# TencentARC/HOSNeRF

Measured on AMD Instinct MI355X. Metric: train rays/sec (stage3: forward + losses + backward + gradient all-reduce + Adam; LPIPS term OFF in this line -- stages.stage3_with_lpips carries it), higher is better.
Workload: dtype f32 (fp16/bf16 hi-lo split MFMA x3, fp32 accumulate)

## Files before the change

hosnerf_amd/csrc/hos_gemm_common.h:

```cpp
#pragma once
#include "hos_common.h"

typedef float f32x16 __attribute__((ext_vector_type(16)));

enum Mode { MODE_FWD = 0, MODE_DGRAD = 1, MODE_WGRAD = 2 };

struct GemmArgs {
    const float* A0; int lda0; int kt0;
    const float* A1; int lda1;
    const float* B;  int ldb;
    float* C; int ldc;
    int M, N;
    int Mload, Nload;
    int red_limit;
    int nk;
    int kt_per_split;
    int tiles_m, tiles_n;
    const float* bias;
    const float* mask; int ldmask;
    float* aux; int aux_col; float p0, p1;
    float* db;
    int accumulate;
    int epi;
    const int* m_dev;
    unsigned int* range_flag;
};

#define HOS_RANGE_LIMIT 6.0e4f


__device__ __forceinline__ bool fwd_epilogue_value(const GemmArgs& a, float& v, int row, int col) {
    switch (a.epi) {
        case HOS_EPI_RELU: v = fmaxf(v, 0.f); break;
        case HOS_EPI_DENSITY: a.aux[row] = softplus_f(v + a.p0); return false;
        case HOS_EPI_RGB: v = sigmoid_f(v) * (1.f + 2.f * a.p0) - a.p0; break;
        case HOS_EPI_NERF_HEAD:
            if (col == a.aux_col) { a.aux[row] = softplus_f(v + a.p0); return false; }
            break;
        case HOS_EPI_SIGMOID_RELU4: v = (col < 3) ? sigmoid_f(v) : fmaxf(v, 0.f); break;
        case HOS_EPI_RESIDUAL: v += a.mask[(size_t)row * a.ldmask + col]; break;
        default: break;
    }
    return true;
}

__device__ __forceinline__ float quad_xor1(float x) {
    return __int_as_float(__builtin_amdgcn_mov_dpp(__float_as_int(x), 0xB1, 0xF, 0xF, true));
}
__device__ __forceinline__ float quad_xor2(float x) {
    return __int_as_float(__builtin_amdgcn_mov_dpp(__float_as_int(x), 0x4E, 0xF, 0xF, true));
}

template <int MODE>
__device__ __forceinline__ void gemm_epilogue_tile(const GemmArgs& a, const f32x16& acc, int row0, int col0, int lane,
                                                   const float4* bias_reg = nullptr, uint32_t* relu_bits = nullptr) {
    const int l31 = lane & 31, lhi = lane >> 5;
    if constexpr (MODE == MODE_WGRAD) {
        const int col = col0 + l31;
        if (col >= a.N) return;
#pragma unroll
        for (int r = 0; r < 16; ++r) {
            const int row = row0 + (r & 3) + 8 * (r >> 2) + 4 * lhi;
            if (row < a.M)
                __hip_atomic_fetch_add(a.C + (size_t)row * a.ldc + col, acc[r], __ATOMIC_RELAXED, __HIP_MEMORY_SCOPE_AGENT);
        }
        return;
    } else {
        const int q = l31 & 3;
        const int colb = col0 + (l31 & ~3);
        const bool c_vec = ((reinterpret_cast<uintptr_t>(a.C) & 15u) == 0) && ((a.ldc & 3) == 0);
        const bool m_vec = a.mask != nullptr && ((reinterpret_cast<uintptr_t>(a.mask) & 15u) == 0) && ((a.ldmask & 3) == 0);
        float4 bias4 = make_float4(0.f, 0.f, 0.f, 0.f);
        bool big = false;
        if (MODE == MODE_FWD && bias_reg != nullptr) bias4 = *bias_reg;
        else if (MODE == MODE_FWD && a.bias != nullptr) {
            if (colb + 0 < a.N) bias4.x = a.bias[colb + 0];
            if (colb + 1 < a.N) bias4.y = a.bias[colb + 1];
            if (colb + 2 < a.N) bias4.z = a.bias[colb + 2];
            if (colb + 3 < a.N) bias4.w = a.bias[colb + 3];
        }
#pragma unroll
        for (int g = 0; g < 4; ++g) {
            float v0 = acc[4 * g + 0], v1 = acc[4 * g + 1], v2 = acc[4 * g + 2], v3 = acc[4 * g + 3];
            {
                const float s0 = (q & 1) ? v0 : v1, s1 = (q & 1) ? v2 : v3;
                const float r0 = quad_xor1(s0), r1 = quad_xor1(s1);
                if (q & 1) { v0 = r0; v2 = r1; } else { v1 = r0; v3 = r1; }
                const float t0 = (q & 2) ? v0 : v2, t1 = (q & 2) ? v1 : v3;
                const float u0 = quad_xor2(t0), u1 = quad_xor2(t1);
                if (q & 2) { v0 = u0; v1 = u1; } else { v2 = u0; v3 = u1; }
            }
            const int row = row0 + q + 8 * g + 4 * lhi;
            if (row >= a.M || colb >= a.N) {
                if (MODE == MODE_FWD && relu_bits != nullptr) *relu_bits <<= 4;
                continue;
            }
            float v[4] = {v0, v1, v2, v3};
            const bool full = colb + 3 < a.N;
            if constexpr (MODE == MODE_FWD) {
                v[0] += bias4.x; v[1] += bias4.y; v[2] += bias4.z; v[3] += bias4.w;
                const bool simple = (a.epi == HOS_EPI_NONE || a.epi == HOS_EPI_RELU);
                if (relu_bits != nullptr) {
                    uint32_t rb = *relu_bits;
#pragma unroll
                    for (int k = 0; k < 4; ++k) rb = __builtin_amdgcn_alignbit(rb, __float_as_uint(0.f - v[k]), 31);
                    *relu_bits = rb;
                }
                if (simple && full && c_vec) {
                    const float pre = (v[0] + v[1]) + (v[2] + v[3]);
                    if (a.epi == HOS_EPI_RELU) { v[0] = fmaxf(v[0], 0.f); v[1] = fmaxf(v[1], 0.f); v[2] = fmaxf(v[2], 0.f); v[3] = fmaxf(v[3], 0.f); }
                    big |= (fmaxf(fmaxf(fabsf(v[0]), fabsf(v[1])), fmaxf(fabsf(v[2]), fabsf(v[3]))) > HOS_RANGE_LIMIT) | (pre != pre);
                    *reinterpret_cast<float4*>(a.C + (size_t)row * a.ldc + colb) = make_float4(v[0], v[1], v[2], v[3]);
                } else {
#pragma unroll
                    for (int k = 0; k < 4; ++k) {
                        const int col = colb + k;
                        if (col >= a.N) break;
                        float x = v[k];
                        if (fwd_epilogue_value(a, x, row, col)) a.C[(size_t)row * a.ldc + col] = x;
                        if (simple) big |= !(fabsf(x) <= HOS_RANGE_LIMIT);
                    }
                }
            } else {
                if (a.mask != nullptr) {
                    if (full && m_vec) {
                        const float4 mk = *reinterpret_cast<const float4*>(a.mask + (size_t)row * a.ldmask + colb);
                        if (!(mk.x > 0.f)) v[0] = 0.f;
                        if (!(mk.y > 0.f)) v[1] = 0.f;
                        if (!(mk.z > 0.f)) v[2] = 0.f;
                        if (!(mk.w > 0.f)) v[3] = 0.f;
                    } else {
#pragma unroll
                        for (int k = 0; k < 4; ++k)
                            if (colb + k < a.N && !(a.mask[(size_t)row * a.ldmask + colb + k] > 0.f)) v[k] = 0.f;
                    }
                }
                float* dst = a.C + (size_t)row * a.ldc + colb;
                if (full && c_vec) {
                    float4 o = make_float4(v[0], v[1], v[2], v[3]);
                    if (a.accumulate) { const float4 p = *reinterpret_cast<const float4*>(dst); o.x += p.x; o.y += p.y; o.z += p.z; o.w += p.w; }
                    *reinterpret_cast<float4*>(dst) = o;
                } else {
#pragma unroll
                    for (int k = 0; k < 4; ++k)
                        if (colb + k < a.N) dst[k] = a.accumulate ? (dst[k] + v[k]) : v[k];
                }
            }
        }
        if (MODE == MODE_FWD && a.range_flag != nullptr && __builtin_amdgcn_ballot_w64(big) != 0 && lane == 0) atomicOr(a.range_flag, 1u);
    }
}

#define HOS_GEMM_FP32 0
#define HOS_GEMM_BF16X3 1
int hos_gemm3_launch(GemmArgs a, int mode, int splits, hipStream_t stream);
```

hosnerf_amd/csrc/hos_mlpbwd.hip:

```cpp
#include "hos_gemm_common.h"
#include <type_traits>
#include <utility>

namespace {

typedef __bf16 bf16x8 __attribute__((ext_vector_type(8)));
typedef __bf16 bf16x4 __attribute__((ext_vector_type(4)));
typedef short s16x4 __attribute__((ext_vector_type(4)));
typedef short s16x8 __attribute__((ext_vector_type(8)));

struct MlpBwdArgs {
    const float* dZ; int lddz;
    const float* X; int ldx;
    const float* W; int ldw;
    float* dX; int lddx;
    float* dW; int lddw;
    float* db;
    int M, N, K;
    int relu_mask;
    float* ws;
    int ws_dw;
    const int* m_dev;
};

constexpr int mb_rows(bool dg) { return dg ? 64 : 32; }
constexpr int MB_NT = 512;

__device__ __forceinline__ float4 ldg4(const float* p) { return *reinterpret_cast<const float4*>(p); }

__device__ __forceinline__ void split4(const float4& v, bf16x4& hi, bf16x4& lo) {
    hi[0] = (__bf16)v.x; hi[1] = (__bf16)v.y; hi[2] = (__bf16)v.z; hi[3] = (__bf16)v.w;
    lo[0] = (__bf16)(v.x - (float)hi[0]); lo[1] = (__bf16)(v.y - (float)hi[1]);
    lo[2] = (__bf16)(v.z - (float)hi[2]); lo[3] = (__bf16)(v.w - (float)hi[3]);
}

__device__ __forceinline__ bf16x8 tr_frag2(const char* p0, int pitch) {
    const s16x4 a = __builtin_amdgcn_ds_read_tr16_b64_v4i16((__attribute__((address_space(3))) s16x4*)(p0));
    const s16x4 b = __builtin_amdgcn_ds_read_tr16_b64_v4i16((__attribute__((address_space(3))) s16x4*)(p0 + 4 * pitch));
    const s16x8 j = __builtin_shufflevector(a, b, 0, 1, 2, 3, 4, 5, 6, 7);
    return __builtin_bit_cast(bf16x8, j);
}

__device__ __forceinline__ f32x16 mma3(const bf16x8& ah, const bf16x8& al, const bf16x8& bh, const bf16x8& bl, f32x16 acc) {
    acc = __builtin_amdgcn_mfma_f32_32x32x16_bf16(al, bh, acc, 0, 0, 0);
    acc = __builtin_amdgcn_mfma_f32_32x32x16_bf16(ah, bl, acc, 0, 0, 0);
    acc = __builtin_amdgcn_mfma_f32_32x32x16_bf16(ah, bh, acc, 0, 0, 0);
    return acc;
}

__device__ __forceinline__ void dgrad_store(const MlpBwdArgs& a, const f32x16& acc, const char* xh_rows, int pitch, int grow0,
                                            int col0, int lane) {
    const int l31 = lane & 31, lhi = lane >> 5, q = l31 & 3;
    const int colb = col0 + (l31 & ~3);
#pragma unroll
    for (int g = 0; g < 4; ++g) {
        float v0 = acc[4 * g + 0], v1 = acc[4 * g + 1], v2 = acc[4 * g + 2], v3 = acc[4 * g + 3];
        {
            const float s0 = (q & 1) ? v0 : v1, s1 = (q & 1) ? v2 : v3;
            const float r0 = quad_xor1(s0), r1 = quad_xor1(s1);
            if (q & 1) { v0 = r0; v2 = r1; } else { v1 = r0; v3 = r1; }
            const float t0 = (q & 2) ? v0 : v2, t1 = (q & 2) ? v1 : v3;
            const float u0 = quad_xor2(t0), u1 = quad_xor2(t1);
            if (q & 2) { v0 = u0; v1 = u1; } else { v2 = u0; v3 = u1; }
        }
        const int lrow = q + 8 * g + 4 * lhi;
        const int row = grow0 + lrow;
        if (row >= a.M || colb >= a.K) continue;
        float v[4] = {v0, v1, v2, v3};
        if (a.relu_mask) {
            const uint2 m = *reinterpret_cast<const uint2*>(xh_rows + lrow * pitch + colb * 2);
            const uint32_t h[4] = {m.x & 0xffffu, m.x >> 16, m.y & 0xffffu, m.y >> 16};
#pragma unroll
            for (int k = 0; k < 4; ++k)
                if ((h[k] & 0x8000u) || (h[k] & 0x7fffu) == 0) v[k] = 0.f;
        }
        float* dst = a.dX + (size_t)row * a.lddx + colb;
        if (colb + 3 < a.K) *reinterpret_cast<float4*>(dst) = make_float4(v[0], v[1], v[2], v[3]);
        else {
#pragma unroll
            for (int k = 0; k < 4; ++k) if (colb + k < a.K) dst[k] = v[k];
        }
    }
}

template <int NT, int KT, bool DG>
__global__ __launch_bounds__(MB_NT, 1) void mlp_bwd_kernel(MlpBwdArgs a) {
    constexpr int N_ = NT * 32, K_ = KT * 32, R = mb_rows(DG);
    if (a.m_dev) a.M = min(a.M, *a.m_dev);
    constexpr int PZ = N_ * 2 + 32, PX = K_ * 2 + 32, PW = K_ * 2 + 32;
    constexpr int W_PLANE = DG ? N_ * PW : 0, Z_PLANE = R * PZ, X_PLANE = R * PX;
    constexpr bool PF2 = DG;
    constexpr int ZU = R * (N_ / 4) / MB_NT, XU = R * (K_ / 4) / MB_NT;
    static_assert(ZU >= 1 && XU >= 1, "tile too small for 512 threads");
    constexpr int DT = DG ? 2 * KT : 0;
    constexpr int WT = NT * KT;
    constexpr int WPW = (WT + 7) / 8;
    static_assert(DT <= 8, "one DGRAD tile per wave");
    static_assert(8 % KT == 0, "a wave's WGRAD tiles share kt");

    extern __shared__ __attribute__((aligned(16))) char smem_mb[];
    char* const Wh = smem_mb;
    char* const Wl = Wh + W_PLANE;
    char* const Zh = Wl + W_PLANE;
    char* const Zl = Zh + Z_PLANE;
    char* const Xh = Zl + Z_PLANE;
    char* const Xl = Xh + X_PLANE;

    const int t = threadIdx.x, lane = t & 63, wave = t >> 6;
    const int l31 = lane & 31, lhi = lane >> 5;
    const int tr_g = lane >> 4, tr_p = lane & 15;
    const int tr_row = 8 * (tr_g >> 1) + (tr_p >> 2);
    const int tr_col = 16 * (tr_g & 1) + 4 * (tr_p & 3);

    float4 rzA[ZU], rxA[XU], rzB[PF2 ? ZU : 1], rxB[PF2 ? XU : 1];
    float4 bsum = make_float4(0.f, 0.f, 0.f, 0.f);
    auto gload = [&](float4 (&rz)[ZU], float4 (&rx)[XU], int rb) {
#pragma unroll
        for (int i = 0; i < ZU; ++i) {
            const int u = t + MB_NT * i, row = u / (N_ / 4), c4 = u % (N_ / 4);
            const int gr = rb * R + row;
            rz[i] = (gr < a.M && c4 * 4 < a.lddz) ? ldg4(a.dZ + (size_t)gr * a.lddz + c4 * 4) : make_float4(0.f, 0.f, 0.f, 0.f);
        }
#pragma unroll
        for (int i = 0; i < XU; ++i) {
            const int u = t + MB_NT * i, row = u / (K_ / 4), c4 = u % (K_ / 4);
            const int gr = rb * R + row;
            rx[i] = (gr < a.M && c4 * 4 < a.K) ? ldg4(a.X + (size_t)gr * a.ldx + c4 * 4) : make_float4(0.f, 0.f, 0.f, 0.f);
        }
    };
    auto sstore = [&](const float4 (&rz)[ZU], const float4 (&rx)[XU]) {
#pragma unroll
        for (int i = 0; i < ZU; ++i) {
            const int u = t + MB_NT * i, row = u / (N_ / 4), c4 = u % (N_ / 4);
            bsum.x += rz[i].x; bsum.y += rz[i].y; bsum.z += rz[i].z; bsum.w += rz[i].w;
            bf16x4 h, l;
            split4(rz[i], h, l);
            *reinterpret_cast<bf16x4*>(Zh + row * PZ + c4 * 8) = h;
            *reinterpret_cast<bf16x4*>(Zl + row * PZ + c4 * 8) = l;
        }
#pragma unroll
        for (int i = 0; i < XU; ++i) {
            const int u = t + MB_NT * i, row = u / (K_ / 4), c4 = u % (K_ / 4);
            bf16x4 h, l;
            split4(rx[i], h, l);
            *reinterpret_cast<bf16x4*>(Xh + row * PX + c4 * 8) = h;
            *reinterpret_cast<bf16x4*>(Xl + row * PX + c4 * 8) = l;
        }
    };

    f32x16 accW[WPW];
#pragma unroll
    for (int j = 0; j < WPW; ++j)
#pragma unroll
        for (int r = 0; r < 16; ++r) accW[j][r] = 0.f;

    const int nrb = (a.M + R - 1) / R;
    const int G = gridDim.x;
    auto compute = [&](int rb) {
        f32x16 acc;
        const int rt = wave / KT, kt = wave % KT;
        if constexpr (DG) if (wave < DT) {
#pragma unroll
            for (int r = 0; r < 16; ++r) acc[r] = 0.f;
            const char* zrow = Zh + (rt * 32 + l31) * PZ + lhi * 16;
            const char* wfrag = Wh + tr_row * PW + (kt * 32 + tr_col) * 2;
#pragma unroll
            for (int s = 0; s < N_ / 16; ++s) {
                const bf16x8 ah = *reinterpret_cast<const bf16x8*>(zrow + s * 32);
                const bf16x8 al = *reinterpret_cast<const bf16x8*>(zrow + Z_PLANE + s * 32);
                const bf16x8 bh = tr_frag2(wfrag + s * 16 * PW, PW);
                const bf16x8 bl = tr_frag2(wfrag + W_PLANE + s * 16 * PW, PW);
                acc = mma3(ah, al, bh, bl, acc);
            }
        }
        if (wave < WT) {
            const int kw = wave % KT;
            const char* xfrag = Xh + tr_row * PX + (kw * 32 + tr_col) * 2;
#pragma unroll
            for (int s = 0; s < R / 16; ++s) {
                const bf16x8 bh = tr_frag2(xfrag + s * 16 * PX, PX);
                const bf16x8 bl = tr_frag2(xfrag + X_PLANE + s * 16 * PX, PX);
#pragma unroll
                for (int j = 0; j < WPW; ++j) {
                    const int ti = wave + 8 * j;
                    if (ti < WT) {
                        const char* zfrag = Zh + tr_row * PZ + ((ti / KT) * 32 + tr_col) * 2;
                        const bf16x8 ah = tr_frag2(zfrag + s * 16 * PZ, PZ);
                        const bf16x8 al = tr_frag2(zfrag + Z_PLANE + s * 16 * PZ, PZ);
                        accW[j] = mma3(ah, al, bh, bl, accW[j]);
                    }
                }
            }
        }
        if constexpr (DG) if (wave < DT && a.dX != nullptr) dgrad_store(a, acc, Xh + rt * 32 * PX, PX, rb * R + rt * 32, kt * 32, lane);
    };

    int rb = blockIdx.x;
    if (rb < nrb) gload(rzA, rxA, rb);
    if constexpr (PF2) if (rb + G < nrb) gload(rzB, rxB, rb + G);
    if constexpr (DG) {
        constexpr int WU = N_ * (K_ / 4) / MB_NT;
        float4 rw[WU];
#pragma unroll
        for (int i = 0; i < WU; ++i) {
            const int u = t + MB_NT * i, row = u / (K_ / 4), c4 = u % (K_ / 4);
            rw[i] = (row < a.N && c4 * 4 < a.K) ? ldg4(a.W + (size_t)row * a.ldw + c4 * 4) : make_float4(0.f, 0.f, 0.f, 0.f);
        }
#pragma unroll
        for (int i = 0; i < WU; ++i) {
            const int u = t + MB_NT * i, row = u / (K_ / 4), c4 = u % (K_ / 4);
            bf16x4 h, l;
            split4(rw[i], h, l);
            *reinterpret_cast<bf16x4*>(Wh + row * PW + c4 * 8) = h;
            *reinterpret_cast<bf16x4*>(Wl + row * PW + c4 * 8) = l;
        }
    }
    if constexpr (PF2) {
        while (rb < nrb) {
            sstore(rzA, rxA);
            __syncthreads();
            if (rb + 2 * G < nrb) gload(rzA, rxA, rb + 2 * G);
            compute(rb);
            __syncthreads();
            rb += G;
            if (rb >= nrb) break;
            sstore(rzB, rxB);
            __syncthreads();
            if (rb + 2 * G < nrb) gload(rzB, rxB, rb + 2 * G);
            compute(rb);
            __syncthreads();
            rb += G;
        }
    } else {
        for (; rb < nrb; rb += G) {
            sstore(rzA, rxA);
            __syncthreads();
            if (rb + G < nrb) gload(rzA, rxA, rb + G);
            compute(rb);
            __syncthreads();
        }
    }

    GemmArgs ew{};
    if (a.ws != nullptr && a.ws_dw) {
        ew.C = a.ws + (size_t)blockIdx.x * (N_ * K_ + N_); ew.ldc = K_; ew.M = N_; ew.N = K_; ew.epi = HOS_EPI_NONE;
#pragma unroll
        for (int j = 0; j < WPW; ++j) {
            const int ti = wave + 8 * j;
            if (ti < WT) gemm_epilogue_tile<MODE_FWD>(ew, accW[j], (ti / KT) * 32, (ti % KT) * 32, lane);
        }
    } else {
        ew.C = a.dW; ew.ldc = a.lddw; ew.M = a.N; ew.N = a.K;
#pragma unroll
        for (int j = 0; j < WPW; ++j) {
            const int ti = wave + 8 * j;
            if (ti < WT) gemm_epilogue_tile<MODE_WGRAD>(ew, accW[j], (ti / KT) * 32, (ti % KT) * 32, lane);
        }
    }
    if (a.db != nullptr) {
        float4* red = reinterpret_cast<float4*>(Zh);
        red[t] = bsum;
        __syncthreads();
        constexpr int G = N_ / 4;
        if (t < G) {
            float4 s = make_float4(0.f, 0.f, 0.f, 0.f);
            for (int k = t; k < MB_NT; k += G) { const float4 v = red[k]; s.x += v.x; s.y += v.y; s.z += v.z; s.w += v.w; }
            const float sv[4] = {s.x, s.y, s.z, s.w};
            bool direct = true;
            if (a.ws != nullptr) {
                const int nk = a.ws_dw ? N_ * K_ : 0;
                *reinterpret_cast<float4*>(a.ws + (size_t)blockIdx.x * (nk + N_) + nk + t * 4) = s;
                direct = false;
            }
            if (direct) {
#pragma unroll
                for (int q = 0; q < 4; ++q)
                    if (t * 4 + q < a.N) __hip_atomic_fetch_add(a.db + t * 4 + q, sv[q], __ATOMIC_RELAXED, __HIP_MEMORY_SCOPE_AGENT);
            }
        }
    }
}

template <int KT>
__global__ __launch_bounds__(MB_NT, 1) void wgrad_tr_fast_kernel(MlpBwdArgs a) {
    constexpr int NT = 8, N_ = NT * 32, K_ = KT * 32, R = 32;
    constexpr int PZ = N_ * 2 + 32, PX = K_ * 2 + 32;
    constexpr int Z_PLANE = R * PZ, X_PLANE = R * PX;
    constexpr int ZU = R * (N_ / 4) / MB_NT;
    constexpr int XT = R * (K_ / 4);
    constexpr int XU = (XT + MB_NT - 1) / MB_NT;
    constexpr bool XALL = XT % MB_NT == 0;
    constexpr int WT = NT * KT, WPW = WT / 8;
    static_assert(WT % 8 == 0 && 8 % KT == 0, "a wave's WGRAD tiles share kt");

    extern __shared__ __attribute__((aligned(16))) char smem_mb[];
    char* const Zh = smem_mb;
    char* const Zl = Zh + Z_PLANE;
    char* const Xh = Zl + Z_PLANE;
    char* const Xl = Xh + X_PLANE;
    const int t = threadIdx.x, lane = t & 63, wave = t >> 6;
    const int tr_g = lane >> 4, tr_p = lane & 15;
    const int tr_row = 8 * (tr_g >> 1) + (tr_p >> 2);
    const int tr_col = 16 * (tr_g & 1) + 4 * (tr_p & 3);
    const bool xthread = XALL || t < XT;

    const int nrb = (a.m_dev ? min(a.M, *a.m_dev) : a.M) / R;
    const int G = gridDim.x;
    float4 rzA[ZU], rxA[XU], rzB[ZU], rxB[XU];
    float4 bsum = make_float4(0.f, 0.f, 0.f, 0.f);
    auto gload = [&](float4 (&rz)[ZU], float4 (&rx)[XU], int rb) {
        rb = rb < nrb ? rb : nrb - 1;
        const float* zb = a.dZ + (size_t)rb * R * a.lddz;
        const float* xb = a.X + (size_t)rb * R * a.ldx;
#pragma unroll
        for (int i = 0; i < ZU; ++i) {
            const int u = t + MB_NT * i, row = u / (N_ / 4), c4 = u % (N_ / 4);
            rz[i] = ldg4(zb + (size_t)row * a.lddz + c4 * 4);
        }
#pragma unroll
        for (int i = 0; i < XU; ++i) {
            const int u = XALL ? t + MB_NT * i : (t < XT ? t : 0), row = u / (K_ / 4), c4 = u % (K_ / 4);
            rx[i] = ldg4(xb + (size_t)row * a.ldx + c4 * 4);
        }
    };
    auto sstore = [&](const float4 (&rz)[ZU], const float4 (&rx)[XU]) {
#pragma unroll
        for (int i = 0; i < ZU; ++i) {
            const int u = t + MB_NT * i, row = u / (N_ / 4), c4 = u % (N_ / 4);
            bsum.x += rz[i].x; bsum.y += rz[i].y; bsum.z += rz[i].z; bsum.w += rz[i].w;
            bf16x4 h, l;
            split4(rz[i], h, l);
            *reinterpret_cast<bf16x4*>(Zh + row * PZ + c4 * 8) = h;
            *reinterpret_cast<bf16x4*>(Zl + row * PZ + c4 * 8) = l;
        }
        if (xthread) {
#pragma unroll
            for (int i = 0; i < XU; ++i) {
                const int u = t + MB_NT * i, row = u / (K_ / 4), c4 = u % (K_ / 4);
                bf16x4 h, l;
                split4(rx[i], h, l);
                *reinterpret_cast<bf16x4*>(Xh + row * PX + c4 * 8) = h;
                *reinterpret_cast<bf16x4*>(Xl + row * PX + c4 * 8) = l;
            }
        }
    };
    f32x16 accW[WPW];
#pragma unroll
    for (int j = 0; j < WPW; ++j)
#pragma unroll
        for (int r = 0; r < 16; ++r) accW[j][r] = 0.f;
    auto compute = [&]() {
        const int kw = wave % KT;
        const char* xfrag = Xh + tr_row * PX + (kw * 32 + tr_col) * 2;
#pragma unroll
        for (int s = 0; s < R / 16; ++s) {
            const bf16x8 bh = tr_frag2(xfrag + s * 16 * PX, PX);
            const bf16x8 bl = tr_frag2(xfrag + X_PLANE + s * 16 * PX, PX);
#pragma unroll
            for (int j = 0; j < WPW; ++j) {
                const int ti = wave + 8 * j;
                const char* zfrag = Zh + tr_row * PZ + ((ti / KT) * 32 + tr_col) * 2;
                const bf16x8 ah = tr_frag2(zfrag + s * 16 * PZ, PZ);
                const bf16x8 al = tr_frag2(zfrag + Z_PLANE + s * 16 * PZ, PZ);
                accW[j] = mma3(ah, al, bh, bl, accW[j]);
            }
        }
    };
#define WG_BAR() asm volatile("s_waitcnt lgkmcnt(0)\n\ts_barrier" ::: "memory")
    auto step = [&](float4 (&rz)[ZU], float4 (&rx)[XU], const int rb) {
        sstore(rz, rx);
        WG_BAR();
        gload(rz, rx, rb + 2 * G);
        compute();
        WG_BAR();
    };
    int rb = blockIdx.x;
    if (rb < nrb) {
        gload(rzA, rxA, rb);
        gload(rzB, rxB, rb + G);
        step(rzA, rxA, rb);
        rb += G;
        if (rb < nrb) {
            step(rzB, rxB, rb);
            rb += G;
            while (rb + G < nrb) {
                step(rzA, rxA, rb);
                step(rzB, rxB, rb + G);
                rb += 2 * G;
            }
            if (rb < nrb) step(rzA, rxA, rb);
        }
    }
#undef WG_BAR
    GemmArgs ew{};
    ew.C = a.ws + (size_t)blockIdx.x * (N_ * K_ + N_); ew.ldc = K_; ew.M = N_; ew.N = K_; ew.epi = HOS_EPI_NONE;
#pragma unroll
    for (int j = 0; j < WPW; ++j) {
        const int ti = wave + 8 * j;
        gemm_epilogue_tile<MODE_FWD>(ew, accW[j], (ti / KT) * 32, (ti % KT) * 32, lane);
    }
    if (a.db != nullptr) {
        float4* red = reinterpret_cast<float4*>(Zh);
        red[t] = bsum;
        __syncthreads();
        constexpr int CG = N_ / 4;
        if (t < CG) {
            float4 sacc = make_float4(0.f, 0.f, 0.f, 0.f);
            for (int k = t; k < MB_NT; k += CG) { const float4 v = red[k]; sacc.x += v.x; sacc.y += v.y; sacc.z += v.z; sacc.w += v.w; }
            *reinterpret_cast<float4*>(a.ws + (size_t)blockIdx.x * (N_ * K_ + N_) + N_ * K_ + t * 4) = sacc;
        }
    }
}

constexpr int MB_RSPLIT = 2;
__global__ __launch_bounds__(256) void mlp_bwd_reduce_kernel(const float* __restrict__ ws, int slabs, int n_, int k_, int nk, float* __restrict__ dW,
                                                             int lddw, float* __restrict__ db, int N, int K) {
    const int e = (blockIdx.x * 256 + threadIdx.x) * 4;
    const int slab = nk + n_;
    if (e >= slab || (e >= nk && db == nullptr)) return;
    float4 s = make_float4(0.f, 0.f, 0.f, 0.f);
    const int sy = gridDim.y;
    for (int g0 = blockIdx.y; g0 < slabs; g0 += 8 * sy) {
        float4 v[8];
#pragma unroll
        for (int i = 0; i < 8; ++i) {
            const int g = g0 + i * sy;
            v[i] = g < slabs ? *reinterpret_cast<const float4*>(ws + (size_t)g * slab + e) : make_float4(0.f, 0.f, 0.f, 0.f);
        }
#pragma unroll
        for (int i = 0; i < 8; ++i) { s.x += v[i].x; s.y += v[i].y; s.z += v[i].z; s.w += v[i].w; }
    }
    const float sv[4] = {s.x, s.y, s.z, s.w};
    if (e >= nk) {
#pragma unroll
        for (int q = 0; q < 4; ++q)
            if (e - nk + q < N) __hip_atomic_fetch_add(db + e - nk + q, sv[q], __ATOMIC_RELAXED, __HIP_MEMORY_SCOPE_AGENT);
        return;
    }
    const int n = e / k_, k = e % k_;
    if (n < N) {
#pragma unroll
        for (int q = 0; q < 4; ++q)
            if (k + q < K) __hip_atomic_fetch_add(dW + (size_t)n * lddw + k + q, sv[q], __ATOMIC_RELAXED, __HIP_MEMORY_SCOPE_AGENT);
    }
}

constexpr int MB_BATCH = 16;
struct ReduceJob { const float* ws; float* dW; float* db; int slabs, n_, k_, nk, lddw, N, K, first_block; };
struct ReduceBatch { ReduceJob j[MB_BATCH]; int count; };

__global__ __launch_bounds__(256) void mlp_bwd_reduce_batch_kernel(const ReduceBatch b) {
    int ji = 0;
#pragma unroll 1
    for (int i = 1; i < b.count; ++i) if ((int)blockIdx.x >= b.j[i].first_block) ji = i;
    const ReduceJob& J = b.j[ji];
    const int e = (((int)blockIdx.x - J.first_block) * 256 + threadIdx.x) * 4;
    const int slab = J.nk + J.n_;
    if (e >= slab || (e >= J.nk && J.db == nullptr)) return;
    float4 s = make_float4(0.f, 0.f, 0.f, 0.f);
    const int sy = gridDim.y;
    for (int g0 = blockIdx.y; g0 < J.slabs; g0 += 8 * sy) {
        float4 v[8];
#pragma unroll
        for (int i = 0; i < 8; ++i) {
            const int g = g0 + i * sy;
            v[i] = g < J.slabs ? *reinterpret_cast<const float4*>(J.ws + (size_t)g * slab + e) : make_float4(0.f, 0.f, 0.f, 0.f);
        }
#pragma unroll
        for (int i = 0; i < 8; ++i) { s.x += v[i].x; s.y += v[i].y; s.z += v[i].z; s.w += v[i].w; }
    }
    const float sv[4] = {s.x, s.y, s.z, s.w};
    if (e >= J.nk) {
#pragma unroll
        for (int q = 0; q < 4; ++q)
            if (e - J.nk + q < J.N) __hip_atomic_fetch_add(J.db + e - J.nk + q, sv[q], __ATOMIC_RELAXED, __HIP_MEMORY_SCOPE_AGENT);
        return;
    }
    const int n = e / J.k_, k = e % J.k_;
    if (n < J.N) {
#pragma unroll
        for (int q = 0; q < 4; ++q)
            if (k + q < J.K) __hip_atomic_fetch_add(J.dW + (size_t)n * J.lddw + k + q, sv[q], __ATOMIC_RELAXED, __HIP_MEMORY_SCOPE_AGENT);
    }
}

thread_local bool g_defer = false;
thread_local ReduceBatch g_batch = {};

static int flush_reduce_batch(hipStream_t stream) {
    if (g_batch.count == 0) return 0;
    const ReduceJob& L = g_batch.j[g_batch.count - 1];
    const int blocks = L.first_block + hos_cdiv(L.nk + L.n_, 1024);
    hipLaunchKernelGGL(mlp_bwd_reduce_batch_kernel, dim3(blocks, MB_RSPLIT), dim3(256), 0, stream, g_batch);
    g_batch.count = 0;
    return hos_launch_status();
}

template <int NT, int KT, bool DG>
int launch_mb(MlpBwdArgs a, size_t ws_floats, hipStream_t stream) {
    constexpr int N_ = NT * 32, K_ = KT * 32;
    constexpr int R = mb_rows(DG);
    constexpr size_t smem = (DG ? 2 * (size_t)N_ * (K_ * 2 + 32) : 0) + 2 * (size_t)R * (N_ * 2 + 32) + 2 * (size_t)R * (K_ * 2 + 32);
    static bool attr_set = false;
    if (!attr_set) {
        hipError_t e = hipFuncSetAttribute(reinterpret_cast<const void*>(&mlp_bwd_kernel<NT, KT, DG>),
                                           hipFuncAttributeMaxDynamicSharedMemorySize, (int)smem);
        if (e != hipSuccess) return (int)e;
        attr_set = true;
    }
    const int nrb = hos_cdiv(a.M, R);
    const int grid = nrb < 256 ? nrb : 256;
    a.ws_dw = 1;
    const int nk = a.ws_dw ? N_ * K_ : 0;
    if (a.ws != nullptr && (grid < 32 || ws_floats < (size_t)grid * (nk + N_) || (!a.ws_dw && a.db == nullptr))) a.ws = nullptr;
    hipLaunchKernelGGL((mlp_bwd_kernel<NT, KT, DG>), dim3(grid), dim3(MB_NT), smem, stream, a);
    if (a.ws != nullptr) {
        if (g_defer) {
            if (g_batch.count == MB_BATCH) { const int rc = flush_reduce_batch(stream); if (rc != 0) return rc; }
            ReduceJob& J = g_batch.j[g_batch.count];
            J = ReduceJob{a.ws, a.dW, a.db, grid, N_, K_, nk, a.lddw, a.N, a.K,
                          g_batch.count ? g_batch.j[g_batch.count - 1].first_block + hos_cdiv(g_batch.j[g_batch.count - 1].nk + g_batch.j[g_batch.count - 1].n_, 1024) : 0};
            ++g_batch.count;
        } else {
            hipLaunchKernelGGL(mlp_bwd_reduce_kernel, dim3(hos_cdiv(nk + N_, 1024), MB_RSPLIT), dim3(256), 0, stream,
                               a.ws, grid, N_, K_, nk, a.dW, a.lddw, a.db, a.N, a.K);
        }
    }
    return hos_launch_status();
}

template <int KT>
int launch_wgrad_fast(MlpBwdArgs a, size_t ws_floats, hipStream_t stream) {
    constexpr int N_ = 256, K_ = KT * 32, R = 32, nk = N_ * K_;
    constexpr size_t smem = 2 * (size_t)R * (N_ * 2 + 32) + 2 * (size_t)R * (K_ * 2 + 32);
    const int nrb = a.M / R;
    const int grid = nrb < 256 ? nrb : 256;
    if (a.M % R != 0 || a.N != N_ || a.K != K_ || a.ws == nullptr || grid < 32 ||
        ws_floats < (size_t)grid * (nk + N_) || (((uintptr_t)a.ws) & 15u)) return -1;
    static bool attr_set = false;
    if (!attr_set) {
        hipError_t e = hipFuncSetAttribute(reinterpret_cast<const void*>(&wgrad_tr_fast_kernel<KT>), hipFuncAttributeMaxDynamicSharedMemorySize, (int)smem);
        if (e != hipSuccess) return (int)e;
        attr_set = true;
    }
    hipLaunchKernelGGL((wgrad_tr_fast_kernel<KT>), dim3(grid), dim3(MB_NT), smem, stream, a);
    if (g_defer) {
        if (g_batch.count == MB_BATCH) { const int rc = flush_reduce_batch(stream); if (rc != 0) return rc; }
        ReduceJob& J = g_batch.j[g_batch.count];
        J = ReduceJob{a.ws, a.dW, a.db, grid, N_, K_, nk, a.lddw, a.N, a.K,
                      g_batch.count ? g_batch.j[g_batch.count - 1].first_block + hos_cdiv(g_batch.j[g_batch.count - 1].nk + g_batch.j[g_batch.count - 1].n_, 1024) : 0};
        ++g_batch.count;
    } else {
        hipLaunchKernelGGL(mlp_bwd_reduce_kernel, dim3(hos_cdiv(nk + N_, 1024), MB_RSPLIT), dim3(256), 0, stream,
                           a.ws, grid, N_, K_, nk, a.dW, a.lddw, a.db, a.N, a.K);
    }
    return hos_launch_status();
}

template <int NT, int KT, bool DG>
int64_t ws_floats_mb(int M) {
    const int nrb = hos_cdiv(M, mb_rows(DG));
    const int grid = nrb < 256 ? nrb : 256;
    return grid < 32 ? 0 : (int64_t)grid * (NT * 32 * KT * 32 + NT * 32);
}


typedef unsigned int u32x4 __attribute__((ext_vector_type(4)));
constexpr int CB_MAXS = 4;
constexpr int CB_R = 64;
constexpr int CB_W_BYTES = 2 * 128 * (128 * 2 + 32);
constexpr int CB_T_BYTES = 2 * CB_R * (128 * 2 + 32);
constexpr int CB_SMEM = CB_W_BYTES + 2 * CB_T_BYTES;

constexpr int cb_code(int nt, int kt, int mask, int out) { return nt | (kt << 4) | (mask << 8) | (out << 9); }
constexpr int cb_nt(int c) { return c & 15; }
constexpr int cb_kt(int c) { return (c >> 4) & 15; }
constexpr bool cb_mask(int c) { return (c >> 8) & 1; }
constexpr bool cb_out(int c) { return (c >> 9) & 1; }
constexpr int cb_image_bytes(int nt, int kt) { return ((2 * nt * 32 * (kt * 64 + 32)) + 8191) / 8192 * 8192; }

struct ChainBwdStep {
    const float* X; int ldx;
    const u32x4* Wp;
    float* dXout; int lddx;
    float* ws;
};
struct ChainBwdArgs {
    const float* dZ; int lddz;
    int M; const int* m_dev;
    ChainBwdStep st[CB_MAXS];
};

template <class F, int... I>
__device__ __forceinline__ void cb_static_for(F&& f, std::integer_sequence<int, I...>) { (f(std::integral_constant<int, I>{}), ...); }

template <int... CODE>
__global__ __launch_bounds__(MB_NT, 1) void chain_bwd_kernel(ChainBwdArgs a) {
    constexpr int S = sizeof...(CODE);
    constexpr int codes[S] = {CODE...};
    static_assert(S >= 1 && S <= CB_MAXS && cb_out(codes[S - 1]), "the last step of a group hands its dX over through HBM");
    constexpr int R = CB_R;
    constexpr auto wpw = [](int s) constexpr { return (cb_nt(codes[s]) * cb_kt(codes[s]) + 7) / 8; };
    constexpr auto acc_off = [wpw](int s) constexpr { int o = 0; for (int i = 0; i < s; ++i) o += wpw(i); return o; };
    constexpr int NACC = acc_off(S);
    constexpr auto zsrc = [](int s) constexpr { int v = -1; for (int i = 0; i < s; ++i) if (!cb_out(codes[i])) v = i; return v; };

    if (a.m_dev) a.M = min(a.M, *a.m_dev);
    extern __shared__ __attribute__((aligned(16))) char smem_mb[];
    char* const Wh = smem_mb;
    char* const Zh = smem_mb + CB_W_BYTES;
    char* const Xh = Zh + CB_T_BYTES;
    const int t = threadIdx.x, lane = t & 63, wave = t >> 6;
    const int l31 = lane & 31, lhi = lane >> 5;
    const int tr_g = lane >> 4, tr_p = lane & 15;
    const int tr_row = 8 * (tr_g >> 1) + (tr_p >> 2);
    const int tr_col = 16 * (tr_g & 1) + 4 * (tr_p & 3);

    constexpr int N0 = cb_nt(codes[0]) * 32;
    constexpr int ZU0 = R * (N0 / 4) / MB_NT;
    float4 rz[ZU0];
    float4 rx[4];
    u32x4 rw[9];
    float4 bsum = make_float4(0.f, 0.f, 0.f, 0.f);
    float4 zsum[S];
    f32x16 accW[NACC];
#pragma unroll
    for (int j = 0; j < NACC; ++j)
#pragma unroll
        for (int r = 0; r < 16; ++r) accW[j][r] = 0.f;
#pragma unroll
    for (int s = 0; s < S; ++s) zsum[s] = make_float4(0.f, 0.f, 0.f, 0.f);

    const int nrb = (a.M + R - 1) / R;
    const int G = gridDim.x;
    const int mlast = a.M - 1;

    auto uni = [](const void* p) {
        const uint64_t v = reinterpret_cast<uint64_t>(p);
        const uint32_t lo = __builtin_amdgcn_readfirstlane((uint32_t)v), hi = __builtin_amdgcn_readfirstlane((uint32_t)(v >> 32));
        return reinterpret_cast<const char*>(((uint64_t)hi << 32) | lo);
    };
    auto blk_rlast = [&](int rb) { return min(R - 1, mlast - rb * R); };
    auto gloadZ = [&](int rb) {
        rb = rb < nrb ? rb : nrb - 1;
        const char* base = uni(a.dZ + (size_t)rb * R * a.lddz);
        const int rlast = blk_rlast(rb);
#pragma unroll
        for (int i = 0; i < ZU0; ++i) {
            const int u = t + MB_NT * i, row = min(u / (N0 / 4), rlast), c4 = u % (N0 / 4);
            rz[i] = *reinterpret_cast<const float4*>(base + (unsigned)((row * a.lddz + c4 * 4) * 4));
        }
    };
    auto sstoreZ = [&](int rb) {
        constexpr int PZ = N0 * 2 + 32;
#pragma unroll
        for (int i = 0; i < ZU0; ++i) {
            const int u = t + MB_NT * i, row = u / (N0 / 4), c4 = u % (N0 / 4);
            float4 v = rz[i];
            if (rb * R + row >= a.M) v = make_float4(0.f, 0.f, 0.f, 0.f);
            bsum.x += v.x; bsum.y += v.y; bsum.z += v.z; bsum.w += v.w;
            bf16x4 h, l;
            split4(v, h, l);
            *reinterpret_cast<bf16x4*>(Zh + row * PZ + c4 * 8) = h;
            *reinterpret_cast<bf16x4*>(Zh + R * PZ + row * PZ + c4 * 8) = l;
        }
    };
    auto gloadX_part = [&](auto sc, int rb, int i0, int i1) {
        constexpr int s = decltype(sc)::value;
        constexpr int K_ = cb_kt(codes[s]) * 32, XU = R * (K_ / 4) / MB_NT;
        rb = rb < nrb ? rb : nrb - 1;
        const int ldx = a.st[s].ldx;
        const char* base = uni(a.st[s].X + (size_t)rb * R * ldx);
        const int rlast = blk_rlast(rb);
#pragma unroll
        for (int i = 0; i < XU; ++i) if (i >= i0 && i < i1) {
            const int u = t + MB_NT * i, row = min(u / (K_ / 4), rlast), c4 = u % (K_ / 4);
            rx[i] = *reinterpret_cast<const float4*>(base + (unsigned)((row * ldx + c4 * 4) * 4));
        }
    };
    auto gloadX = [&](auto sc, int rb) { gloadX_part(sc, rb, 0, 4); };
    auto sstoreX = [&](auto sc) {
        constexpr int s = decltype(sc)::value;
        constexpr int K_ = cb_kt(codes[s]) * 32, XU = R * (K_ / 4) / MB_NT, PX = K_ * 2 + 32;
#pragma unroll
        for (int i = 0; i < XU; ++i) {
            const int u = t + MB_NT * i, row = u / (K_ / 4), c4 = u % (K_ / 4);
            bf16x4 h, l;
            split4(rx[i], h, l);
            *reinterpret_cast<bf16x4*>(Xh + row * PX + c4 * 8) = h;
            *reinterpret_cast<bf16x4*>(Xh + R * PX + row * PX + c4 * 8) = l;
        }
    };
    const unsigned toff = (unsigned)t * 16u;
    auto loadW_part = [&](auto sc, int i0, int i1) {
        constexpr int s = decltype(sc)::value;
        constexpr int RW = cb_image_bytes(cb_nt(codes[s]), cb_kt(codes[s])) / 8192;
#pragma unroll
        for (int i = 0; i < RW; ++i) if (i >= i0 && i < i1) rw[i] = *reinterpret_cast<const u32x4*>(uni(reinterpret_cast<const char*>(a.st[s].Wp) + (size_t)i * 8192) + toff);
// ... 120 lines not shown
                    if (wave < DT) {
                        const int q = l31 & 3;
                        const int colb = kt * 32 + (l31 & ~3);
#pragma unroll
                        for (int g = 0; g < 4; ++g) {
                            const int lrow = rt * 32 + q + 8 * g + 4 * lhi;
                            bf16x4 h, l;
                            split4(make_float4(v[g][0], v[g][1], v[g][2], v[g][3]), h, l);
                            *reinterpret_cast<bf16x4*>(Zh + lrow * PZn + colb * 2) = h;
                            *reinterpret_cast<bf16x4*>(Zh + R * PZn + lrow * PZn + colb * 2) = l;
                        }
                    }
                }
                sstoreX(std::integral_constant<int, s + 1 < S ? s + 1 : 0>{});
                storeW(std::integral_constant<int, s + 1 < S ? s + 1 : 0>{});
                __syncthreads();
            }
        }, std::make_integer_sequence<int, S>{});
        __syncthreads();
    }

    cb_static_for([&](auto sc) {
        constexpr int s = decltype(sc)::value;
        constexpr int NT = cb_nt(codes[s]), KT = cb_kt(codes[s]), N_ = NT * 32, K_ = KT * 32;
        constexpr int WT = NT * KT, WPW = (WT + 7) / 8;
        GemmArgs ew{};
        ew.C = a.st[s].ws + (size_t)blockIdx.x * (N_ * K_ + N_); ew.ldc = K_; ew.M = N_; ew.N = K_; ew.epi = HOS_EPI_NONE;
#pragma unroll
        for (int j = 0; j < WPW; ++j) {
            const int ti = wave + 8 * j;
            if (ti < WT) gemm_epilogue_tile<MODE_FWD>(ew, accW[acc_off(s) + j], (ti / KT) * 32, (ti % KT) * 32, lane);
        }
    }, std::make_integer_sequence<int, S>{});
    float4* red = reinterpret_cast<float4*>(Zh);
    {
        red[t] = bsum;
        __syncthreads();
        constexpr int CG = N0 / 4;
        float4 sacc = make_float4(0.f, 0.f, 0.f, 0.f);
        if (t < CG)
            for (int k = t; k < MB_NT; k += CG) { const float4 x = red[k]; sacc.x += x.x; sacc.y += x.y; sacc.z += x.z; sacc.w += x.w; }
        cb_static_for([&](auto sc) {
            constexpr int s = decltype(sc)::value;
            constexpr int N_ = cb_nt(codes[s]) * 32, K_ = cb_kt(codes[s]) * 32;
            if constexpr (zsrc(s) == -1)
                if (t < CG) *reinterpret_cast<float4*>(a.st[s].ws + (size_t)blockIdx.x * (N_ * K_ + N_) + N_ * K_ + t * 4) = sacc;
        }, std::make_integer_sequence<int, S>{});
        __syncthreads();
    }
    cb_static_for([&](auto pc) {
        constexpr int p = decltype(pc)::value;
        if constexpr (!cb_out(codes[p])) {
            constexpr int KTp = cb_kt(codes[p]), CG = KTp * 8;
            red[t] = (wave < 2 * KTp) ? zsum[p] : make_float4(0.f, 0.f, 0.f, 0.f);
            __syncthreads();
            float4 sacc = make_float4(0.f, 0.f, 0.f, 0.f);
            if (t < CG) {
                const int kt = t >> 3, cq = t & 7;
#pragma unroll
                for (int rt = 0; rt < 2; ++rt)
#pragma unroll
                    for (int hh = 0; hh < 2; ++hh)
#pragma unroll
                        for (int q = 0; q < 4; ++q) {
                            const float4 x = red[(rt * KTp + kt) * 64 + hh * 32 + cq * 4 + q];
                            sacc.x += x.x; sacc.y += x.y; sacc.z += x.z; sacc.w += x.w;
                        }
            }
            cb_static_for([&](auto sc) {
                constexpr int s = decltype(sc)::value;
                constexpr int N_ = cb_nt(codes[s]) * 32, K_ = cb_kt(codes[s]) * 32;
                if constexpr (zsrc(s) == p)
                    if (t < CG) *reinterpret_cast<float4*>(a.st[s].ws + (size_t)blockIdx.x * (N_ * K_ + N_) + N_ * K_ + t * 4) = sacc;
            }, std::make_integer_sequence<int, S>{});
            __syncthreads();
        }
    }, std::make_integer_sequence<int, S>{});
}

struct ChainBwdPackJob { const float* W; int ldw, N, K, nt, kt; uint16_t* image; };
struct ChainBwdPackJobs { ChainBwdPackJob j[8]; };
__global__ __launch_bounds__(256) void chain_bwd_pack_kernel(const ChainBwdPackJobs jobs) {
    const ChainBwdPackJob& J = jobs.j[blockIdx.y];
    const int N_ = J.nt * 32, K_ = J.kt * 32, pw = K_ + 16;
    const int total = cb_image_bytes(J.nt, J.kt) / 2;
    for (int e = blockIdx.x * 256 + threadIdx.x; e < total; e += gridDim.x * 256) {
        const int plane = e / (N_ * pw), r = e % (N_ * pw);
        const int n = r / pw, k = r % pw;
        uint16_t out = 0;
        if (plane < 2 && n < J.N && k < J.K) {
            const float w = J.W[(size_t)n * J.ldw + k];
            const __bf16 hi = (__bf16)w;
            out = plane == 0 ? __builtin_bit_cast(uint16_t, hi) : __builtin_bit_cast(uint16_t, (__bf16)(w - (float)hi));
        }
        J.image[e] = out;
    }
}

struct ChainBwdCfg { int S; int code[CB_MAXS]; };
constexpr int CB_NCFG = 4;
constexpr ChainBwdCfg CB_CFG[CB_NCFG] = {
    {2, {cb_code(1, 4, 1, 0), cb_code(4, 4, 1, 1), 0, 0}},
    {3, {cb_code(4, 2, 0, 1), cb_code(4, 4, 1, 0), cb_code(4, 4, 1, 1), 0}},
    {3, {cb_code(4, 4, 1, 0), cb_code(4, 4, 1, 0), cb_code(4, 2, 0, 1), 0}},
    {3, {cb_code(4, 4, 1, 0), cb_code(4, 4, 1, 0), cb_code(4, 4, 0, 1), 0}},
};

template <int... CODE>
int launch_chain_bwd(const ChainBwdArgs& a, int grid, hipStream_t stream) {
    static bool attr_set = false;
    if (!attr_set) {
        hipError_t e = hipFuncSetAttribute(reinterpret_cast<const void*>(&chain_bwd_kernel<CODE...>), hipFuncAttributeMaxDynamicSharedMemorySize, CB_SMEM);
        if (e != hipSuccess) return (int)e;
        attr_set = true;
    }
    hipLaunchKernelGGL((chain_bwd_kernel<CODE...>), dim3(grid), dim3(MB_NT), CB_SMEM, stream, a);
    return hos_launch_status();
}

}

extern "C" int hos_linear_bwd_fused(const float* dZ, int lddz, const float* X, int ldx, const float* W, int ldw,
                                    float* dX, int lddx, float* dW, int lddw, float* db, int M, int N, int K,
                                    int relu_mask, float* ws, int64_t ws_floats, const int32_t* rows_dev, hos_stream_t stream) {
    if (!dZ || !X || !W || !dW || M <= 0 || N <= 0 || K <= 0 || ws_floats < 0) return HOS_E_ARG;
    if (N > 128 || K > 128) return HOS_E_SHAPE;
    if ((lddz & 3) || (ldx & 3) || (ldw & 3) || (K & 3) || (dX && (lddx & 3))) return HOS_E_ALIGN;
    if (((uintptr_t)dZ | (uintptr_t)X | (uintptr_t)W | (uintptr_t)ws) & 15u) return HOS_E_ALIGN;
    MlpBwdArgs a{dZ, lddz, X, ldx, W, ldw, dX, lddx, dW, lddw, db, M, N, K, relu_mask, ws, 1, rows_dev};
    hipStream_t s = static_cast<hipStream_t>(stream);
    const int nt = hos_cdiv(N, 32), kt = hos_cdiv(K, 32);
    if (nt <= 1 && kt <= 4) return launch_mb<1, 4, true>(a, (size_t)ws_floats, s);
    if (kt <= 2) return launch_mb<4, 2, true>(a, (size_t)ws_floats, s);
    return launch_mb<4, 4, true>(a, (size_t)ws_floats, s);
}

extern "C" int hos_linear_wgrad_tr(const float* dZ, int lddz, const float* X, int ldx, float* dW, int lddw, float* db,
                                   int M, int N, int K, float* ws, int64_t ws_floats, const int32_t* rows_dev, hos_stream_t stream) {
    if (!dZ || !X || !dW || M <= 0 || N <= 0 || K <= 0) return HOS_E_ARG;
    if (N > 256 || K > 256) return HOS_E_SHAPE;
    if ((lddz & 3) || (ldx & 3) || (K & 3)) return HOS_E_ALIGN;
    if (((uintptr_t)dZ | (uintptr_t)X) & 15u) return HOS_E_ALIGN;
    MlpBwdArgs a{dZ, lddz, X, ldx, nullptr, 0, nullptr, 0, dW, lddw, db, M, N, K, 0, ws, 0, rows_dev};
    hipStream_t s = static_cast<hipStream_t>(stream);
    const int kt = hos_cdiv(K, 32);
    if (N == 256 && (K == 256 || K == 64)) {
        const int rc = K == 256 ? launch_wgrad_fast<8>(a, (size_t)ws_floats, s) : launch_wgrad_fast<2>(a, (size_t)ws_floats, s);
        if (rc >= 0) return rc;
    }
    if (kt <= 4) return launch_mb<8, 4, false>(a, (size_t)ws_floats, s);
    return launch_mb<8, 8, false>(a, (size_t)ws_floats, s);
}

extern "C" int hos_mlp_bwd_defer(int on) { g_defer = on != 0; return 0; }

extern "C" int hos_mlp_bwd_flush(hos_stream_t stream) { return flush_reduce_batch(static_cast<hipStream_t>(stream)); }

extern "C" long long hos_mlp_bwd_ws_floats(int M, int N, int K, int fused) {
    if (M <= 0 || N <= 0 || K <= 0) return 0;
    const int nt = hos_cdiv(N, 32), kt = hos_cdiv(K, 32);
    if (fused) {
        if (nt <= 1 && kt <= 4) return ws_floats_mb<1, 4, true>(M);
        if (kt <= 2) return ws_floats_mb<4, 2, true>(M);
        return ws_floats_mb<4, 4, true>(M);
    }
    return kt <= 4 ? ws_floats_mb<8, 4, false>(M) : ws_floats_mb<8, 8, false>(M);
}

extern "C" int hos_mlp_chain_bwd_steps(int cfg) { return cfg >= 0 && cfg < CB_NCFG ? CB_CFG[cfg].S : HOS_E_ARG; }

extern "C" long long hos_mlp_chain_bwd_image_bytes(int cfg, int step) {
    if (cfg < 0 || cfg >= CB_NCFG || step < 0 || step >= CB_CFG[cfg].S) return 0;
    return cb_image_bytes(cb_nt(CB_CFG[cfg].code[step]), cb_kt(CB_CFG[cfg].code[step]));
}

extern "C" long long hos_mlp_chain_bwd_ws_floats(int cfg, int M) {
    if (cfg < 0 || cfg >= CB_NCFG || M <= 0) return 0;
    const int nrb = hos_cdiv(M, CB_R), grid = nrb < 256 ? nrb : 256;
    long long f = 0;
    for (int s = 0; s < CB_CFG[cfg].S; ++s) {
        const int n_ = cb_nt(CB_CFG[cfg].code[s]) * 32, k_ = cb_kt(CB_CFG[cfg].code[s]) * 32;
        f += (long long)grid * (n_ * k_ + n_);
    }
    return f;
}

extern "C" int hos_mlp_chain_bwd_pack(int n, const int* cfg, const int* step, const float* const* W, const int* ldw, const int* N,
                                      const int* K, void* const* image, hos_stream_t stream) {
    if (n <= 0 || n > 8 || !cfg || !step || !W || !ldw || !N || !K || !image) return HOS_E_ARG;
    ChainBwdPackJobs jobs{};
    for (int i = 0; i < n; ++i) {
        if (cfg[i] < 0 || cfg[i] >= CB_NCFG || step[i] < 0 || step[i] >= CB_CFG[cfg[i]].S || !W[i] || !image[i] || N[i] <= 0 || K[i] <= 0) return HOS_E_ARG;
        const int nt = cb_nt(CB_CFG[cfg[i]].code[step[i]]), kt = cb_kt(CB_CFG[cfg[i]].code[step[i]]);
        if (N[i] > nt * 32 || K[i] > kt * 32 || ldw[i] < K[i]) return HOS_E_SHAPE;
        if ((uintptr_t)image[i] & 15u) return HOS_E_ALIGN;
        jobs.j[i] = ChainBwdPackJob{W[i], ldw[i], N[i], K[i], nt, kt, static_cast<uint16_t*>(image[i])};
    }
    hipLaunchKernelGGL(chain_bwd_pack_kernel, dim3(36, n), dim3(256), 0, static_cast<hipStream_t>(stream), jobs);
    return hos_launch_status();
}

extern "C" int hos_mlp_chain_bwd(int cfg, const float* dZ, int lddz, int M, const int32_t* rows_dev, const float* const* X, const int* ldx,
                                 const void* const* images, float* const* dXout, const int* lddx, float* const* dW, const int* lddw,
                                 float* const* db, const int* N, const int* K, float* ws, int64_t ws_floats, hos_stream_t stream) {
    if (cfg < 0 || cfg >= CB_NCFG || !dZ || M <= 0 || !X || !ldx || !images || !dXout || !lddx || !dW || !lddw || !db || !N || !K || !ws) return HOS_E_ARG;
    const ChainBwdCfg& C = CB_CFG[cfg];
    if (ws_floats < hos_mlp_chain_bwd_ws_floats(cfg, M)) return HOS_E_SHAPE;
    if (((uintptr_t)dZ | (uintptr_t)ws) & 15u) return HOS_E_ALIGN;
    if (lddz < cb_nt(C.code[0]) * 32 || (lddz & 3)) return HOS_E_SHAPE;
    const int nrb = hos_cdiv(M, CB_R), grid = nrb < 256 ? nrb : 256;
    ChainBwdArgs a{};
    a.dZ = dZ; a.lddz = lddz; a.M = M; a.m_dev = rows_dev;
    float* wsp = ws;
    ReduceJob jobs[CB_MAXS];
    for (int s = 0; s < C.S; ++s) {
        const int n_ = cb_nt(C.code[s]) * 32, k_ = cb_kt(C.code[s]) * 32;
        if (!X[s] || !images[s] || !dW[s] || N[s] <= 0 || K[s] <= 0 || N[s] > n_ || K[s] > k_) return HOS_E_ARG;
        if (ldx[s] < k_ || (ldx[s] & 3) || (((uintptr_t)X[s] | (uintptr_t)images[s]) & 15u)) return HOS_E_ALIGN;
        if (cb_out(C.code[s])) {
            if (!dXout[s] || lddx[s] < k_ || (lddx[s] & 3) || ((uintptr_t)dXout[s] & 15u)) return HOS_E_ALIGN;
        }
        a.st[s].X = X[s]; a.st[s].ldx = ldx[s]; a.st[s].Wp = static_cast<const u32x4*>(images[s]);
        a.st[s].dXout = dXout[s]; a.st[s].lddx = lddx[s]; a.st[s].ws = wsp;
        jobs[s] = ReduceJob{wsp, dW[s], db[s], grid, n_, k_, n_ * k_, lddw[s], N[s], K[s], 0};
        wsp += (size_t)grid * (n_ * k_ + n_);
    }
    hipStream_t st = static_cast<hipStream_t>(stream);
    int rc;
    switch (cfg) {
        case 0: rc = launch_chain_bwd<CB_CFG[0].code[0], CB_CFG[0].code[1]>(a, grid, st); break;
        case 1: rc = launch_chain_bwd<CB_CFG[1].code[0], CB_CFG[1].code[1], CB_CFG[1].code[2]>(a, grid, st); break;
        case 2: rc = launch_chain_bwd<CB_CFG[2].code[0], CB_CFG[2].code[1], CB_CFG[2].code[2]>(a, grid, st); break;
        default: rc = launch_chain_bwd<CB_CFG[3].code[0], CB_CFG[3].code[1], CB_CFG[3].code[2]>(a, grid, st); break;
    }
    if (rc != 0) return rc;
    for (int s = 0; s < C.S; ++s) {
        if (g_defer) {
            if (g_batch.count == MB_BATCH) { const int r2 = flush_reduce_batch(st); if (r2 != 0) return r2; }
            ReduceJob& J = g_batch.j[g_batch.count];
            J = jobs[s];
            J.first_block = g_batch.count ? g_batch.j[g_batch.count - 1].first_block + hos_cdiv(g_batch.j[g_batch.count - 1].nk + g_batch.j[g_batch.count - 1].n_, 1024) : 0;
            ++g_batch.count;
        } else {
            const ReduceJob& J = jobs[s];
            hipLaunchKernelGGL(mlp_bwd_reduce_kernel, dim3(hos_cdiv(J.nk + J.n_, 1024), MB_RSPLIT), dim3(256), 0, st,
                               J.ws, J.slabs, J.n_, J.k_, J.nk, J.dW, J.lddw, J.db, J.N, J.K);
        }
    }
    return hos_launch_status();
}
```

hosnerf_amd/csrc/hos_thin.hip:

```cpp
#include "hos_gemm_common.h"
#include <type_traits>

namespace {

constexpr int TH_PF2_MAXKS = 16;
constexpr int TH_R_FWD = 32;

template <typename E> struct V8 { typedef E t __attribute__((ext_vector_type(8))); typedef E q __attribute__((ext_vector_type(4))); };

__device__ __forceinline__ f32x16 mfma_e(const V8<__bf16>::t& a, const V8<__bf16>::t& b, const f32x16& c) {
    return __builtin_amdgcn_mfma_f32_32x32x16_bf16(a, b, c, 0, 0, 0);
}
__device__ __forceinline__ f32x16 mfma_e(const V8<_Float16>::t& a, const V8<_Float16>::t& b, const f32x16& c) {
    return __builtin_amdgcn_mfma_f32_32x32x16_f16(a, b, c, 0, 0, 0);
}
template <typename E> __device__ __forceinline__ float hi_of(float x) { return x; }
template <> __device__ __forceinline__ float hi_of<_Float16>(float x) { return __builtin_amdgcn_fmed3f(x, -65504.f, 65504.f); }

template <typename E>
__device__ __forceinline__ void split_pair(float x, E& hi, E& lo) {
    hi = (E)hi_of<E>(x);
    lo = (E)(x - (float)hi);
}

struct ThinArgs {
    const float* A; int lda;
    const float* W; int ldw;
    const float* bias;
    float* C; int ldc;
    int M, N, K;
    int epi;
    const float* mask; int ldmask;
    unsigned int* range_flag;
    uint16_t* bits;
    const int* m_dev;
};

__device__ __forceinline__ int th_live_tiles(const ThinArgs& a) { return (a.m_dev ? min(a.M, *a.m_dev) : a.M) / 32; }

constexpr int TH_NT = 512;
constexpr int TH_PAD_DGRAD = 16, TH_PAD_FWD = 32;
template <bool DGRAD> constexpr int th_pad() { return DGRAD ? TH_PAD_DGRAD : TH_PAD_FWD; }
constexpr int TH_MP = 264;
__device__ __forceinline__ float4 ld4(const float* p) { return *reinterpret_cast<const float4*>(p); }

template <int KS, bool DGRAD>
__global__ __launch_bounds__(TH_NT, 1) void thin_gemm_kernel(ThinArgs a) {
    if (a.m_dev) a.M = min(a.M, *a.m_dev);
    typedef typename std::conditional<DGRAD, __bf16, _Float16>::type E;
    typedef typename V8<E>::t e8;
    typedef typename V8<E>::q e4;
    constexpr int R = DGRAD ? 32 : TH_R_FWD;
    constexpr int KD = KS * 16;
    constexpr int P = KD * 2 + th_pad<DGRAD>();
    constexpr int PLANE = R * P, BUF = 2 * PLANE;
    constexpr int MSK = DGRAD ? R * TH_MP : 0;
    constexpr int AU = R * (KD / 4) / TH_NT;
    constexpr int MU = DGRAD ? R * 64 / TH_NT : 1;
    static_assert(AU >= 1, "tile too small");

    extern __shared__ __attribute__((aligned(16))) char smem_th[];
    char* const buf0 = smem_th;
    char* const msk0 = smem_th + 2 * BUF;

    const int t = threadIdx.x, lane = t & 63, wave = t >> 6;
    const int l31 = lane & 31, lhi = lane >> 5;
    const int col0 = wave * 32;

    e8 bh[KS], bl[KS];
    {
        const int j = col0 + l31;
#pragma unroll
        for (int s = 0; s < KS; ++s) {
            float w[8];
            const int k0 = 16 * s + 8 * lhi;
#pragma unroll
            for (int q = 0; q < 8; ++q) w[q] = 0.f;
            if (j < a.N) {
                if constexpr (!DGRAD) {
                    if (k0 + 7 < a.K) {
                        const float4 u = ld4(a.W + (size_t)j * a.ldw + k0), v = ld4(a.W + (size_t)j * a.ldw + k0 + 4);
                        w[0] = u.x; w[1] = u.y; w[2] = u.z; w[3] = u.w; w[4] = v.x; w[5] = v.y; w[6] = v.z; w[7] = v.w;
                    } else {
#pragma unroll
                        for (int q = 0; q < 8; ++q) if (k0 + q < a.K) w[q] = a.W[(size_t)j * a.ldw + k0 + q];
                    }
                } else {
#pragma unroll
                    for (int q = 0; q < 8; ++q) if (k0 + q < a.K) w[q] = a.W[(size_t)(k0 + q) * a.ldw + j];
                }
            }
#pragma unroll
            for (int q = 0; q < 8; ++q) { E h, l; split_pair<E>(w[q], h, l); bh[s][q] = h; bl[s][q] = l; }
        }
    }

    const int msh = (int)((reinterpret_cast<uintptr_t>(a.mask) >> 2) & 3u);
    const float* const mbase = a.mask - msh;
    float4 ra[AU], rm[MU], rmx = make_float4(0.f, 0.f, 0.f, 0.f);
    uint32_t rbits = 0, bits_staged = 0, bits_cur = 0;
    auto gload = [&](int tile) {
#pragma unroll
        for (int i = 0; i < AU; ++i) {
            const int u = t + TH_NT * i, row = u / (KD / 4), c4 = u % (KD / 4);
            const int gr = tile * R + row;
            ra[i] = (gr < a.M && c4 * 4 < a.K) ? ld4(a.A + (size_t)gr * a.lda + c4 * 4) : make_float4(0.f, 0.f, 0.f, 0.f);
        }
        if constexpr (DGRAD) {
            if (a.bits != nullptr) rbits = a.bits[(size_t)tile * TH_NT + t];
            else if (a.mask != nullptr) {
#pragma unroll
                for (int i = 0; i < MU; ++i) {
                    const int u = t + TH_NT * i, row = u >> 6, c4 = u & 63;
                    const int gr = tile * R + row;
                    rm[i] = (gr < a.M && c4 * 4 < a.N + msh) ? ld4(mbase + (size_t)gr * a.ldmask + c4 * 4) : make_float4(0.f, 0.f, 0.f, 0.f);
                }
                if (msh != 0 && t < R) {
                    const int gr = tile * R + t;
                    rmx = (gr < a.M && 256 < a.N + msh) ? ld4(mbase + (size_t)gr * a.ldmask + 256) : make_float4(0.f, 0.f, 0.f, 0.f);
                }
            }
        }
    };
    auto sstore = [&](int b) {
        char* const hi = buf0 + b * BUF;
        char* const lo = hi + PLANE;
#pragma unroll
        for (int i = 0; i < AU; ++i) {
            const int u = t + TH_NT * i, row = u / (KD / 4), c4 = u % (KD / 4);
            e4 h, l;
            const float xs[4] = {ra[i].x, ra[i].y, ra[i].z, ra[i].w};
#pragma unroll
            for (int q = 0; q < 4; ++q) { E hh, ll; split_pair<E>(xs[q], hh, ll); h[q] = hh; l[q] = ll; }
            *reinterpret_cast<e4*>(hi + row * P + c4 * 8) = h;
            *reinterpret_cast<e4*>(lo + row * P + c4 * 8) = l;
        }
        if constexpr (DGRAD) {
            if (a.bits != nullptr) bits_staged = rbits;
            else if (a.mask != nullptr) {
#pragma unroll
                for (int i = 0; i < MU; ++i) {
                    const int u = t + TH_NT * i, row = u >> 6, c4 = u & 63;
                    const uint32_t m = (rm[i].x > 0.f ? 1u : 0u) | (rm[i].y > 0.f ? 0x100u : 0u) | (rm[i].z > 0.f ? 0x10000u : 0u) |
                                       (rm[i].w > 0.f ? 0x1000000u : 0u);
                    *reinterpret_cast<uint32_t*>(msk0 + b * MSK + row * TH_MP + c4 * 4) = m;
                }
                if (msh != 0 && t < R) {
                    const uint32_t m = (rmx.x > 0.f ? 1u : 0u) | (rmx.y > 0.f ? 0x100u : 0u) | (rmx.z > 0.f ? 0x10000u : 0u) |
                                       (rmx.w > 0.f ? 0x1000000u : 0u);
                    *reinterpret_cast<uint32_t*>(msk0 + b * MSK + t * TH_MP + 256) = m;
                }
            }
        }
    };

    GemmArgs ef{};
    ef.C = a.C; ef.ldc = a.ldc; ef.M = a.M; ef.N = a.N; ef.bias = a.bias; ef.epi = a.epi; ef.range_flag = a.range_flag;
    float4 bias4 = make_float4(0.f, 0.f, 0.f, 0.f);
    if (!DGRAD && a.bias != nullptr) {
        const int cb = col0 + (l31 & ~3);
        if (cb + 0 < a.N) bias4.x = a.bias[cb + 0];
        if (cb + 1 < a.N) bias4.y = a.bias[cb + 1];
        if (cb + 2 < a.N) bias4.z = a.bias[cb + 2];
        if (cb + 3 < a.N) bias4.w = a.bias[cb + 3];
    }

    const int ntiles = (a.M + R - 1) / R;
    const int G = gridDim.x;
    int tile = blockIdx.x;
    if (tile < ntiles) { gload(tile); sstore(0); }
    if (tile + G < ntiles) gload(tile + G);
    __syncthreads();
    int b = 0;
    for (; tile < ntiles; tile += G, b ^= 1) {
        const bool more = tile + G < ntiles;
        if constexpr (DGRAD) bits_cur = bits_staged;
        const char* hi = buf0 + b * BUF + l31 * P + lhi * 16;
        f32x16 acc[R / 32];
#pragma unroll
        for (int rt = 0; rt < R / 32; ++rt)
#pragma unroll
            for (int r = 0; r < 16; ++r) acc[rt][r] = 0.f;
#pragma unroll
        for (int s = 0; s < KS; ++s) {
#pragma unroll
            for (int rt = 0; rt < R / 32; ++rt) {
                const e8 ah = *reinterpret_cast<const e8*>(hi + rt * 32 * P + s * 32);
                const e8 al = *reinterpret_cast<const e8*>(hi + PLANE + rt * 32 * P + s * 32);
                acc[rt] = mfma_e(al, bh[s], acc[rt]);
                acc[rt] = mfma_e(ah, bl[s], acc[rt]);
                acc[rt] = mfma_e(ah, bh[s], acc[rt]);
            }
        }
        if (more) sstore(b ^ 1);
        if (tile + 2 * G < ntiles) gload(tile + 2 * G);
        if (col0 < a.N) {
#pragma unroll
            for (int rt = 0; rt < R / 32; ++rt) {
                const int row0 = tile * R + rt * 32;
                if constexpr (!DGRAD) {
                    uint32_t rb = 0;
                    gemm_epilogue_tile<MODE_FWD>(ef, acc[rt], row0, col0, lane, &bias4, &rb);
                    if (a.bits != nullptr) a.bits[((size_t)tile * (R / 32) + rt) * TH_NT + t] = (uint16_t)rb;
                } else {
                    const int q = l31 & 3, colb = col0 + (l31 & ~3);
#pragma unroll
                    for (int g = 0; g < 4; ++g) {
                        float v0 = acc[rt][4 * g + 0], v1 = acc[rt][4 * g + 1], v2 = acc[rt][4 * g + 2], v3 = acc[rt][4 * g + 3];
                        {
                            const float s0 = (q & 1) ? v0 : v1, s1 = (q & 1) ? v2 : v3;
                            const float r0 = quad_xor1(s0), r1 = quad_xor1(s1);
                            if (q & 1) { v0 = r0; v2 = r1; } else { v1 = r0; v3 = r1; }
                            const float t0 = (q & 2) ? v0 : v2, t1 = (q & 2) ? v1 : v3;
                            const float u0 = quad_xor2(t0), u1 = quad_xor2(t1);
                            if (q & 2) { v0 = u0; v1 = u1; } else { v2 = u0; v3 = u1; }
                        }
                        const int lrow = q + 8 * g + 4 * lhi, row = row0 + lrow;
                        if (row >= a.M || colb >= a.N) continue;
                        float v[4] = {v0, v1, v2, v3};
                        if (a.bits != nullptr) {
#pragma unroll
                            for (int k = 0; k < 4; ++k)
                                v[k] = __uint_as_float(__float_as_uint(v[k]) & (uint32_t)__builtin_amdgcn_sbfe((int)bits_cur, 15 - (4 * g + k), 1));
                        } else if (a.mask != nullptr) {
                            const char* const mp = msk0 + b * MSK + (rt * 32 + lrow) * TH_MP + colb;
                            uint32_t m = *reinterpret_cast<const uint32_t*>(mp);
                            if (msh != 0) m = __builtin_amdgcn_alignbyte(*reinterpret_cast<const uint32_t*>(mp + 4), m, (uint32_t)msh);
#pragma unroll
                            for (int k = 0; k < 4; ++k) if (!((m >> (8 * k)) & 1u)) v[k] = 0.f;
                        }
                        float* dst = a.C + (size_t)row * a.ldc + colb;
                        if (colb + 3 < a.N && ((reinterpret_cast<uintptr_t>(dst) & 15u) == 0)) *reinterpret_cast<float4*>(dst) = make_float4(v[0], v[1], v[2], v[3]);
                        else {
#pragma unroll
                            for (int k = 0; k < 4; ++k) if (colb + k < a.N) dst[k] = v[k];
                        }
                    }
                }
            }
        }
        __syncthreads();
    }
}

template <int KS, bool BITS>
__global__ __launch_bounds__(TH_NT, 1) void thin_fwd_fast_kernel(const ThinArgs a) {
    typedef _Float16 E;
    typedef typename V8<E>::t e8;
    typedef typename V8<E>::q e4;
    constexpr int R = 32;
    const int ntiles = th_live_tiles(a);
    if ((int)blockIdx.x >= ntiles) return;
    constexpr int KD = KS * 16;
    constexpr int P = KD * 2 + TH_PAD_FWD;
    constexpr int PLANE = R * P, BUF = 2 * PLANE;
    constexpr int AU = R * (KD / 4) / TH_NT;
    constexpr bool PF2 = KS <= TH_PF2_MAXKS;
    constexpr int PFD = PF2 ? 3 : 2;
    static_assert(AU >= 1 && R * (KD / 4) % TH_NT == 0, "tile does not divide over 512 threads");

    extern __shared__ __attribute__((aligned(16))) char smem_th[];
    char* const buf0 = smem_th;
    const int t = threadIdx.x, lane = t & 63, wave = t >> 6;
    const int l31 = lane & 31, lhi = lane >> 5;
    const int col0 = wave * 32;

    e8 bh[KS], bl[KS];
    {
        const float* wrow = a.W + (size_t)(col0 + l31) * a.ldw + 8 * lhi;
#pragma unroll
        for (int s = 0; s < KS; ++s) {
            const float4 u = ld4(wrow + 16 * s), v = ld4(wrow + 16 * s + 4);
            const float w[8] = {u.x, u.y, u.z, u.w, v.x, v.y, v.z, v.w};
#pragma unroll
            for (int q = 0; q < 8; ++q) { E h, l; split_pair<E>(w[q], h, l); bh[s][q] = h; bl[s][q] = l; }
        }
    }
    const int q4 = l31 & 3, colb = col0 + (l31 & ~3);
    const float4 bias4 = a.bias != nullptr ? ld4(a.bias + colb) : make_float4(0.f, 0.f, 0.f, 0.f);
    const bool relu = a.epi == HOS_EPI_RELU;

    const int G = gridDim.x;
    float4 ra[AU], rb[PF2 ? AU : 1];
    auto gload = [&](float4 (&r)[AU], int tile) {
        tile = tile < ntiles ? tile : ntiles - 1;
        const float* base = a.A + (size_t)tile * R * a.lda;
#pragma unroll
        for (int i = 0; i < AU; ++i) {
            const int u = t + TH_NT * i, row = u / (KD / 4), c4 = u % (KD / 4);
            r[i] = ld4(base + (size_t)row * a.lda + c4 * 4);
        }
    };
    auto sstore = [&](const float4 (&r)[AU], int b) {
        char* const hi = buf0 + b * BUF;
        char* const lo = hi + PLANE;
#pragma unroll
        for (int i = 0; i < AU; ++i) {
            const int u = t + TH_NT * i, row = u / (KD / 4), c4 = u % (KD / 4);
            e4 h, l;
            const float xs[4] = {r[i].x, r[i].y, r[i].z, r[i].w};
#pragma unroll
            for (int q = 0; q < 4; ++q) { E hh, ll; split_pair<E>(xs[q], hh, ll); h[q] = hh; l[q] = ll; }
            *reinterpret_cast<e4*>(hi + row * P + c4 * 8) = h;
            *reinterpret_cast<e4*>(lo + row * P + c4 * 8) = l;
        }
    };

    int tile = blockIdx.x;
    gload(ra, tile);
    sstore(ra, 0);
    gload(ra, tile + G);
    if constexpr (PF2) gload(rb, tile + 2 * G);
    __syncthreads();
    bool big = false;
    auto body = [&](float4 (&rcur)[AU], const int tile, const int b, const bool more) {
        const char* hi = buf0 + b * BUF + l31 * P + lhi * 16;
        f32x16 acc;
#pragma unroll
        for (int r = 0; r < 16; ++r) acc[r] = 0.f;
#pragma unroll
        for (int s = 0; s < KS; ++s) {
            const e8 ah = *reinterpret_cast<const e8*>(hi + s * 32);
            const e8 al = *reinterpret_cast<const e8*>(hi + PLANE + s * 32);
            acc = mfma_e(al, bh[s], acc);
            acc = mfma_e(ah, bl[s], acc);
            acc = mfma_e(ah, bh[s], acc);
        }
        if (more) sstore(rcur, b ^ 1);
        gload(rcur, tile + PFD * G);
        uint32_t rbits = 0;
        float* crow = a.C + (size_t)(tile * R + q4 + 4 * lhi) * a.ldc + colb;
#pragma unroll
        for (int g = 0; g < 4; ++g) {
            float v0 = acc[4 * g + 0], v1 = acc[4 * g + 1], v2 = acc[4 * g + 2], v3 = acc[4 * g + 3];
            {
                const float s0 = (q4 & 1) ? v0 : v1, s1 = (q4 & 1) ? v2 : v3;
                const float r0 = quad_xor1(s0), r1 = quad_xor1(s1);
                if (q4 & 1) { v0 = r0; v2 = r1; } else { v1 = r0; v3 = r1; }
                const float t0 = (q4 & 2) ? v0 : v2, t1 = (q4 & 2) ? v1 : v3;
                const float u0 = quad_xor2(t0), u1 = quad_xor2(t1);
                if (q4 & 2) { v0 = u0; v1 = u1; } else { v2 = u0; v3 = u1; }
            }
            float v[4] = {v0 + bias4.x, v1 + bias4.y, v2 + bias4.z, v3 + bias4.w};
            if constexpr (BITS) {
                uint32_t m = 0;
#pragma unroll
                for (int k = 0; k < 4; ++k) m = __builtin_amdgcn_alignbit(m, __float_as_uint(0.f - v[k]), 31);
                rbits |= m << (12 - 4 * g);
            }
            const float pre = (v[0] + v[1]) + (v[2] + v[3]);
            if (relu) { v[0] = fmaxf(v[0], 0.f); v[1] = fmaxf(v[1], 0.f); v[2] = fmaxf(v[2], 0.f); v[3] = fmaxf(v[3], 0.f); }
            big |= (fmaxf(fmaxf(fabsf(v[0]), fabsf(v[1])), fmaxf(fabsf(v[2]), fabsf(v[3]))) > HOS_RANGE_LIMIT) | (pre != pre);
            *reinterpret_cast<float4*>(crow + (size_t)(8 * g) * a.ldc) = make_float4(v[0], v[1], v[2], v[3]);
        }
        if constexpr (BITS) {
            const uint32_t odd = (uint32_t)__builtin_amdgcn_mov_dpp((int)rbits, 0xB1, 0xF, 0xF, true);
            if ((lane & 1) == 0) reinterpret_cast<uint32_t*>(a.bits)[((size_t)tile * TH_NT + t) >> 1] = (rbits & 0xffffu) | (odd << 16);
        }
        asm volatile("s_waitcnt lgkmcnt(0)\n\ts_barrier" ::: "memory");
    };
    int b = 0;
    if constexpr (PF2) {
        body(ra, tile, b, tile + G < ntiles);
        tile += G; b ^= 1;
        if (tile < ntiles) {
            body(rb, tile, b, tile + G < ntiles);
            tile += G; b ^= 1;
            while (tile + G < ntiles) {
                body(ra, tile, b, true);
                body(rb, tile + G, b ^ 1, tile + 2 * G < ntiles);
                tile += 2 * G;
            }
            if (tile < ntiles) body(ra, tile, b, false);
        }
    } else {
        body(ra, tile, b, tile + G < ntiles);
        tile += G; b ^= 1;
        for (; tile < ntiles; tile += G, b ^= 1) body(ra, tile, b, tile + G < ntiles);
    }
    if (a.range_flag != nullptr && __builtin_amdgcn_ballot_w64(big) != 0 && lane == 0) atomicOr(a.range_flag, 1u);
}

template <bool MASK>
__global__ __launch_bounds__(TH_NT, 1) void thin_dgrad_fast_kernel(const ThinArgs a) {
    typedef __bf16 E;
    typedef typename V8<E>::t e8;
    typedef typename V8<E>::q e4;
    constexpr int KS = 16, R = 32;
    const int ntiles = th_live_tiles(a);
    if ((int)blockIdx.x >= ntiles) return;
    constexpr int KD = KS * 16;
    constexpr int P = KD * 2 + th_pad<true>();
    constexpr int PLANE = R * P, BUF = 2 * PLANE;
    constexpr int AU = R * (KD / 4) / TH_NT;
    constexpr int PFD = 3;

    extern __shared__ __attribute__((aligned(16))) char smem_th[];
    char* const buf0 = smem_th;
    const int t = threadIdx.x, lane = t & 63, wave = t >> 6;
    const int l31 = lane & 31, lhi = lane >> 5;
    const int col0 = wave * 32;

    const bool active = col0 < a.N;
    e8 bh[KS], bl[KS];
    if (active) {
        const float* wcol = a.W + (size_t)(8 * lhi) * a.ldw + col0 + l31;
#pragma unroll
        for (int s = 0; s < KS; ++s)
#pragma unroll
            for (int q = 0; q < 8; ++q) { E h, l; split_pair<E>(wcol[(size_t)(16 * s + q) * a.ldw], h, l); bh[s][q] = h; bl[s][q] = l; }
    }
    const int q4 = l31 & 3, colb = col0 + (l31 & ~3);
    const int G = gridDim.x;
    float4 ra[AU], rb[AU];
    uint32_t ba = 0, bb = 0, bits_staged = 0;
    auto gload = [&](float4 (&r)[AU], uint32_t& rbits, int tile) {
        tile = tile < ntiles ? tile : ntiles - 1;
        const float* base = a.A + (size_t)tile * R * a.lda;
#pragma unroll
        for (int i = 0; i < AU; ++i) {
            const int u = t + TH_NT * i, row = u / (KD / 4), c4 = u % (KD / 4);
            r[i] = ld4(base + (size_t)row * a.lda + c4 * 4);
        }
        if constexpr (MASK) rbits = a.bits[(size_t)tile * TH_NT + t];
    };
    auto sstore = [&](const float4 (&r)[AU], const uint32_t rbits, int b) {
        char* const hi = buf0 + b * BUF;
        char* const lo = hi + PLANE;
#pragma unroll
        for (int i = 0; i < AU; ++i) {
            const int u = t + TH_NT * i, row = u / (KD / 4), c4 = u % (KD / 4);
            e4 h, l;
            const float xs[4] = {r[i].x, r[i].y, r[i].z, r[i].w};
#pragma unroll
            for (int q = 0; q < 4; ++q) { E hh, ll; split_pair<E>(xs[q], hh, ll); h[q] = hh; l[q] = ll; }
            *reinterpret_cast<e4*>(hi + row * P + c4 * 8) = h;
            *reinterpret_cast<e4*>(lo + row * P + c4 * 8) = l;
        }
        bits_staged = rbits;
    };

    int tile = blockIdx.x;
    gload(ra, ba, tile);
    sstore(ra, ba, 0);
    gload(ra, ba, tile + G);
    gload(rb, bb, tile + 2 * G);
    __syncthreads();
    auto body = [&](auto act, float4 (&rcur)[AU], uint32_t& bcur, const int tile, const int b, const bool more) {
        constexpr bool ACT = decltype(act)::value;
        const uint32_t bits_cur = bits_staged;
        const char* hi = buf0 + b * BUF + l31 * P + lhi * 16;
        f32x16 acc;
        if constexpr (ACT) {
#pragma unroll
            for (int r = 0; r < 16; ++r) acc[r] = 0.f;
#pragma unroll
            for (int s = 0; s < KS; ++s) {
                const e8 ah = *reinterpret_cast<const e8*>(hi + s * 32);
                const e8 al = *reinterpret_cast<const e8*>(hi + PLANE + s * 32);
                acc = mfma_e(al, bh[s], acc);
                acc = mfma_e(ah, bl[s], acc);
                acc = mfma_e(ah, bh[s], acc);
            }
        }
        if (more) sstore(rcur, bcur, b ^ 1);
        gload(rcur, bcur, tile + PFD * G);
        float* crow = a.C + (size_t)(tile * R + q4 + 4 * lhi) * a.ldc + colb;
        if constexpr (ACT)
#pragma unroll
        for (int g = 0; g < 4; ++g) {
            float v0 = acc[4 * g + 0], v1 = acc[4 * g + 1], v2 = acc[4 * g + 2], v3 = acc[4 * g + 3];
            {
                const float s0 = (q4 & 1) ? v0 : v1, s1 = (q4 & 1) ? v2 : v3;
                const float r0 = quad_xor1(s0), r1 = quad_xor1(s1);
                if (q4 & 1) { v0 = r0; v2 = r1; } else { v1 = r0; v3 = r1; }
                const float t0 = (q4 & 2) ? v0 : v2, t1 = (q4 & 2) ? v1 : v3;
                const float u0 = quad_xor2(t0), u1 = quad_xor2(t1);
                if (q4 & 2) { v0 = u0; v1 = u1; } else { v2 = u0; v3 = u1; }
            }
            float v[4] = {v0, v1, v2, v3};
            if constexpr (MASK) {
#pragma unroll
                for (int k = 0; k < 4; ++k)
                    v[k] = __uint_as_float(__float_as_uint(v[k]) & (uint32_t)__builtin_amdgcn_sbfe((int)bits_cur, 15 - (4 * g + k), 1));
            }
            *reinterpret_cast<float4*>(crow + (size_t)(8 * g) * a.ldc) = make_float4(v[0], v[1], v[2], v[3]);
        }
        asm volatile("s_waitcnt lgkmcnt(0)\n\ts_barrier" ::: "memory");
    };
    auto run = [&](auto act) {
        int b = 0;
        body(act, ra, ba, tile, b, tile + G < ntiles);
        tile += G; b ^= 1;
        if (tile < ntiles) {
            body(act, rb, bb, tile, b, tile + G < ntiles);
            tile += G; b ^= 1;
            while (tile + G < ntiles) {
                body(act, ra, ba, tile, b, true);
                body(act, rb, bb, tile + G, b ^ 1, tile + 2 * G < ntiles);
                tile += 2 * G;
            }
            if (tile < ntiles) body(act, ra, ba, tile, b, false);
        }
    };
    if (active) run(std::true_type{});
    else run(std::false_type{});
}

template <bool MASK>
int launch_thin_dgrad_fast(const ThinArgs& a, hipStream_t stream) {
    constexpr size_t smem = 2 * 2 * (size_t)32 * (16 * 32 + th_pad<true>());
    static bool attr_set = false;
    if (!attr_set) {
        hipError_t e = hipFuncSetAttribute(reinterpret_cast<const void*>(&thin_dgrad_fast_kernel<MASK>),
                                           hipFuncAttributeMaxDynamicSharedMemorySize, (int)smem);
        if (e != hipSuccess) return (int)e;
        attr_set = true;
    }
    const int ntiles = a.M / 32;
    const int grid = ntiles < 256 ? ntiles : 256;
    hipLaunchKernelGGL((thin_dgrad_fast_kernel<MASK>), dim3(grid), dim3(TH_NT), smem, stream, a);
    return hos_launch_status();
}

template <int KS, bool BITS>
int launch_thin_fast(const ThinArgs& a, hipStream_t stream) {
    constexpr size_t smem = 2 * 2 * (size_t)32 * (KS * 32 + TH_PAD_FWD);
    static bool attr_set = false;
    if (!attr_set) {
        hipError_t e = hipFuncSetAttribute(reinterpret_cast<const void*>(&thin_fwd_fast_kernel<KS, BITS>),
                                           hipFuncAttributeMaxDynamicSharedMemorySize, (int)smem);
        if (e != hipSuccess) return (int)e;
        attr_set = true;
    }
    const int ntiles = a.M / 32;
    const int grid = ntiles < 256 ? ntiles : 256;
    hipLaunchKernelGGL((thin_fwd_fast_kernel<KS, BITS>), dim3(grid), dim3(TH_NT), smem, stream, a);
    return hos_launch_status();
}

template <int KS, bool DGRAD>
int launch_thin(const ThinArgs& a, hipStream_t stream) {
    constexpr int R = DGRAD ? 32 : TH_R_FWD;
    constexpr size_t smem = 2 * 2 * (size_t)R * (KS * 32 + th_pad<DGRAD>()) + (DGRAD ? 2 * (size_t)R * TH_MP : 0);
    static bool attr_set = false;
    if (!attr_set) {
        hipError_t e = hipFuncSetAttribute(reinterpret_cast<const void*>(&thin_gemm_kernel<KS, DGRAD>),
                                           hipFuncAttributeMaxDynamicSharedMemorySize, (int)smem);
        if (e != hipSuccess) return (int)e;
        attr_set = true;
    }
    const int ntiles = hos_cdiv(a.M, R);
    const int grid = ntiles < 256 ? ntiles : 256;
    hipLaunchKernelGGL((thin_gemm_kernel<KS, DGRAD>), dim3(grid), dim3(TH_NT), smem, stream, a);
    return hos_launch_status();
}

struct CnlFold {
    const float* W0; int ld0; const float* b0; const float* W5; int ld5; const float* b5;
    const float* embed; int n0, nf, ne, nh, nfp;
    float* W0f; float* b0f; float* W5f; float* b5f;
    float* gW0; float* gb0; float* gW5; float* gb5; float* g_embed;
};

__global__ __launch_bounds__(256) void cnl_fold_pack_kernel(const CnlFold a) {
    const int n = blockIdx.x, t = threadIdx.x;
    const float* w0 = a.W0 + (size_t)n * a.ld0;
    const float* w5 = a.W5 + (size_t)n * a.ld5;
    for (int k = t; k < a.nfp; k += 256) a.W0f[(size_t)n * a.nfp + k] = k < a.nf ? w0[k] : 0.f;
    const int k5 = a.nfp + a.nh;
    for (int k = t; k < k5; k += 256) a.W5f[(size_t)n * k5 + k] = k < a.nf ? w5[k] : (k < a.nfp ? 0.f : w5[a.nf + a.ne + (k - a.nfp)]);
    if (t < 2) {
        const float* w = (t ? w5 : w0) + a.nf;
        float v = t ? a.b5[n] : a.b0[n];
        for (int c = 0; c < a.ne; ++c) v = fmaf(w[c], a.embed[c], v);
        (t ? a.b5f : a.b0f)[n] = v;
    }
}

__global__ __launch_bounds__(256) void cnl_fold_unfold_kernel(const CnlFold a) {
    const int t = threadIdx.x;
    if ((int)blockIdx.x >= a.n0) {
        __shared__ float part[256];
        const int c = (int)blockIdx.x - a.n0;
        float s = 0.f;
        for (int n = t; n < a.n0; n += 256) s = fmaf(a.W0[(size_t)n * a.ld0 + a.nf + c], a.b0f[n], s);
        for (int n = t; n < a.n0; n += 256) s = fmaf(a.W5[(size_t)n * a.ld5 + a.nf + c], a.b5f[n], s);
        part[t] = s;
        __syncthreads();
        for (int w = 128; w > 0; w >>= 1) {
            if (t < w) part[t] += part[t + w];
            __syncthreads();
        }
        if (t == 0) a.g_embed[c] += part[0];
        return;
    }
    const int n = blockIdx.x;
    const float d0 = a.b0f[n], d5 = a.b5f[n];
    float* g0 = a.gW0 + (size_t)n * a.ld0;
    float* g5 = a.gW5 + (size_t)n * a.ld5;
    const int k5 = a.nfp + a.nh;
    for (int k = t; k < a.nf + a.ne; k += 256) {
        g0[k] += k < a.nf ? a.W0f[(size_t)n * a.nfp + k] : d0 * a.embed[k - a.nf];
        g5[k] += k < a.nf ? a.W5f[(size_t)n * k5 + k] : d5 * a.embed[k - a.nf];
    }
    for (int j = t; j < a.nh; j += 256) g5[a.nf + a.ne + j] += a.W5f[(size_t)n * k5 + a.nfp + j];
    if (t == 0) { a.gb0[n] += d0; a.gb5[n] += d5; }
}

}

extern "C" int hos_canonical_fold_pack(const float* W0, int ld0, const float* b0, const float* W5, int ld5, const float* b5,
                                       const float* embed, int n_out, int nf, int ne, int nh,
                                       float* W0f, float* b0f, float* W5f, float* b5f, hos_stream_t stream) {
    if (!W0 || !b0 || !W5 || !b5 || !embed || !W0f || !b0f || !W5f || !b5f) return HOS_E_ARG;
    if (n_out <= 0 || nf <= 0 || ne <= 0 || nh <= 0 || ld0 < nf + ne || ld5 < nf + ne + nh) return HOS_E_SHAPE;
    CnlFold a{W0, ld0, b0, W5, ld5, b5, embed, n_out, nf, ne, nh, (nf + 3) & ~3, W0f, b0f, W5f, b5f, nullptr, nullptr, nullptr, nullptr, nullptr};
    hipLaunchKernelGGL(cnl_fold_pack_kernel, dim3(n_out), dim3(256), 0, static_cast<hipStream_t>(stream), a);
    return hos_launch_status();
}

extern "C" int hos_canonical_fold_unfold(const float* gW0f, const float* db0, const float* gW5f, const float* db5,
                                         const float* W0, int ld0, const float* W5, int ld5, const float* embed,
                                         int n_out, int nf, int ne, int nh,
                                         float* gW0, float* gb0, float* gW5, float* gb5, float* g_embed, hos_stream_t stream) {
    if (!gW0f || !db0 || !gW5f || !db5 || !W0 || !W5 || !embed || !gW0 || !gb0 || !gW5 || !gb5 || !g_embed) return HOS_E_ARG;
    if (n_out <= 0 || nf <= 0 || ne <= 0 || ne > 256 || nh <= 0 || ld0 < nf + ne || ld5 < nf + ne + nh) return HOS_E_SHAPE;
    CnlFold a{W0, ld0, nullptr, W5, ld5, nullptr, embed, n_out, nf, ne, nh, (nf + 3) & ~3,
              const_cast<float*>(gW0f), const_cast<float*>(db0), const_cast<float*>(gW5f), const_cast<float*>(db5), gW0, gb0, gW5, gb5, g_embed};
    hipLaunchKernelGGL(cnl_fold_unfold_kernel, dim3(n_out + ne), dim3(256), 0, static_cast<hipStream_t>(stream), a);
    return hos_launch_status();
}

extern "C" int hos_thin_linear_fwd(const float* X, int ldx, const float* W, int ldw, const float* bias, float* Y, int ldy,
                                   int M, int N, int K, int epilogue, void* relu_bits, const int32_t* rows_dev, hos_stream_t stream) {
    if (!X || !W || !Y || M <= 0 || N <= 0 || K <= 0) return HOS_E_ARG;
    if (N > 256 || K > 320 || (epilogue != HOS_EPI_NONE && epilogue != HOS_EPI_RELU)) return HOS_E_SHAPE;
    if ((ldx & 3) || (ldw & 3) || (K & 3) || (((uintptr_t)X | (uintptr_t)W) & 15u)) return HOS_E_ALIGN;
    if (relu_bits && ((uintptr_t)relu_bits & 1u)) return HOS_E_ALIGN;
    ThinArgs a{X, ldx, W, ldw, bias, Y, ldy, M, N, K, epilogue, nullptr, 0, hos_range_flag_ptr(), static_cast<uint16_t*>(relu_bits), rows_dev};
    hipStream_t s = static_cast<hipStream_t>(stream);
    if (N == 256 && M >= 32 && (K == 64 || K == 256 || K == 320) && !(ldy & 3) && !((uintptr_t)Y & 15u) &&
        (!bias || !((uintptr_t)bias & 15u)) && !((uintptr_t)relu_bits & 3u) && (!rows_dev || !(M & 31))) {
        ThinArgs f = a;
        f.M = M & ~31;
        int rc;
        if (relu_bits) rc = K == 64 ? launch_thin_fast<4, true>(f, s) : (K == 256 ? launch_thin_fast<16, true>(f, s) : launch_thin_fast<20, true>(f, s));
        else rc = K == 64 ? launch_thin_fast<4, false>(f, s) : (K == 256 ? launch_thin_fast<16, false>(f, s) : launch_thin_fast<20, false>(f, s));
        if (rc != 0 || f.M == M) return rc;
        a.A += (size_t)f.M * ldx; a.C += (size_t)f.M * ldy; a.M = M - f.M;
        if (a.bits) a.bits += (size_t)(f.M / 32) * TH_NT;
    }
    if (K <= 64) return launch_thin<4, false>(a, s);
    if (K <= 128) return launch_thin<8, false>(a, s);
    return K <= 256 ? launch_thin<16, false>(a, s) : launch_thin<20, false>(a, s);
}

extern "C" int hos_thin_linear_dgrad(const float* dY, int lddy, const float* W, int ldw, int Npad, const float* mask, int ldmask,
                                     const void* mask_bits, float* dX, int lddx, int M, int K, const int32_t* rows_dev,
                                     hos_stream_t stream) {
    if (!dY || !W || !dX || M <= 0 || K <= 0 || Npad <= 0) return HOS_E_ARG;
    if (K > 256 || Npad > 256) return HOS_E_SHAPE;
    if ((lddy & 3) || (Npad & 3) || (mask && (ldmask & 3)) || ((uintptr_t)dY & 15u) || (((uintptr_t)W | (uintptr_t)mask) & 3u)) return HOS_E_ALIGN;
    if (mask_bits && ((uintptr_t)mask_bits & 1u)) return HOS_E_ALIGN;
    ThinArgs a{dY, lddy, W, ldw, nullptr, dX, lddx, M, K, Npad, 0, mask_bits ? nullptr : mask, ldmask, nullptr,
               static_cast<uint16_t*>(const_cast<void*>(mask_bits)), rows_dev};
    hipStream_t s = static_cast<hipStream_t>(stream);
    if ((K == 256 || K == 64) && Npad == 256 && M >= 32 && (mask_bits || !mask) && !(lddx & 3) && !((uintptr_t)dX & 15u) &&
        (!rows_dev || !(M & 31))) {
        ThinArgs f = a;
        f.M = M & ~31;
        const int rc = mask_bits ? launch_thin_dgrad_fast<true>(f, s) : launch_thin_dgrad_fast<false>(f, s);
        if (rc != 0 || f.M == M) return rc;
        a.A += (size_t)f.M * lddy; a.C += (size_t)f.M * lddx; a.M = M - f.M;
        if (a.bits) a.bits += (size_t)(f.M / 32) * TH_NT;
    }
    return Npad <= 128 ? launch_thin<8, true>(a, s) : launch_thin<16, true>(a, s);
}
```

hosnerf_amd/human_nerf.py:

```python
from __future__ import annotations

import json
import math
import os
from types import SimpleNamespace
from typing import Dict, List, Optional

import numpy as np
import torch
import torch.nn as nn
import torch.nn.functional as F

from . import ops
from .flat import FlatModule, FlatStore, Region
from .mipnerf360 import select_state, _Lin

SMPL_PARENT = {1: 0, 2: 0, 3: 0, 4: 1, 5: 2, 6: 3, 7: 4, 8: 5, 9: 6, 10: 7, 11: 8, 12: 9, 13: 9, 14: 9, 15: 12,
               16: 13, 17: 14, 18: 16, 19: 17, 20: 18, 21: 19, 22: 20, 23: 21, 24: 23, 25: 22}


class Cfg(dict):

    def __getattr__(self, k):
        try:
# ... 326 lines not shown
    def decoder_shard_spans(self):
        out = []
        if self.decoder_shard is not None:
            for n in self._shard_layers:
                off, row, cin = self._shard_rows(n)
                cs = cin // self.decoder_shard.world
                out.append((off + self.decoder_shard.rank * cs * row, cs * row))
        return out

    @torch.no_grad()
    def gather_decoder_shards(self, optimizer=None):
        comm = self.decoder_shard
        if comm is None:
            return
        flats = [self.flat_param]
        for f in (getattr(optimizer, "fused", None) or ([optimizer] if optimizer is not None else [])):
            if getattr(f, "module", None) is self:
                flats += [f.exp_avg, f.exp_avg_sq]
        for n in self._shard_layers:
            off, row, cin = self._shard_rows(n)
            cs = cin // comm.world
            for flat in flats:
                mine = flat[off + comm.rank * cs * row: off + (comm.rank + 1) * cs * row]
                flat[off: off + cin * row].copy_(comm.all_gather(mine).reshape(-1))

    split_decoder_backward = False
    _pending_vol = None
    _fwd_stream = None

    def lazy_param_spans(self):
        spans = [(self._embeds.offset + k * 64, 64) for k in range(len(self.human_stateembeds))]
        first = self._plain["pose_decoder.block_mlps.0.weight"]
        lo = (first.data_ptr() - self.flat_param.data_ptr()) // 4
        spans.append((int(lo), int(self._nr[0].W.offset - lo)))
        return spans

    def decoder_span(self):
        first = self._plain["pose_decoder.block_mlps.0.weight"]
        off = (first.data_ptr() - self.flat_param.data_ptr()) // 4
        return 0, int(off)

    def pending_volume_grad(self):
        return None if self._pending_vol is None else self._pending_vol[1].grad

    def finish_decoder_backward(self):
        pend, self._pending_vol = self._pending_vol, None
        if pend is not None and pend[1].grad is not None:
            pend[0].backward(pend[1].grad)
            fs = self._fwd_stream
            if fs is not None and pend[0].is_cuda and fs != torch.cuda.current_stream(pend[0].device):
                torch.cuda.current_stream(pend[0].device).wait_stream(fs)

    def decoder_backward(self, group=None):
        g = self.pending_volume_grad()
        if g is not None:
            import torch.distributed as dist
            if dist.is_available() and dist.is_initialized() and dist.get_world_size(group) > 1:
                dist.all_reduce(g, group=group)
        self.finish_decoder_backward()

    def reduce_ranges(self):
        off, n = self.decoder_span()
        return [(off + n, self.flat_param.numel() - off - n)]

    def _band_weights(self, iter_val: float, device) -> torch.Tensor:
        c = self.cfg.non_rigid_motion_mlp
        kick = torch.tensor(float(c.kick_in_iter), dtype=torch.float32)
        t = torch.clamp(torch.tensor(float(iter_val), dtype=torch.float32) - kick, min=0.0)
        Nn = c.full_band_iter - kick
        alpha = c.multires * t / Nn
        j = torch.arange(c.multires, dtype=torch.float32)
        w = (1.0 - torch.cos(np.pi * torch.clamp(alpha - j, min=0.0, max=1.0))) / 2.0
        key = (tuple(w.tolist()), str(device))
        cache = getattr(self, "_band_cache", None)
        if cache is None or cache[0] != key:
            self._band_cache = (key, w.to(device))
        return self._band_cache[1]

    def _nonrigid_fwd(self, specs: List[_LayerSpec], x: torch.Tensor, cond: torch.Tensor, band_w: torch.Tensor, save: bool, rows_dev=None):
        Pn = x.shape[0]
        dev = x.device
        PE = torch.empty(Pn, NR_LDPE, device=dev)
        chain = ops.MLP_CHAIN and Pn >= ops.MLP_CHAIN_MIN_ROWS and ops.get_gemm_mode() != ops.GEMM_FP32
        if chain and ops.MLP_CHAIN_FOLD:
            cond = cond.reshape(-1).contiguous()
            ops.embed_hannw(x, band_w, None, PE, rows_dev=rows_dev)
            key = (id(specs),) + ops._stream_key(dev)
            bufs = self._chain_bufs.get(key)
            if bufs is None or len(bufs) < 3:
                bufs = self._chain_bufs[key] = ops.mlp_chain_buffers(dev) + (torch.empty(128, 64, device=dev),)
            ws = [self._w(L) for L in specs]
            ops.mlp_chain_pack_fold([w for w, _ in ws], [b_ for _, b_ in ws], cond, 6 * band_w.numel(), bufs[0], bufs[1], bufs[2])
            acts = [torch.empty(Pn, 128, device=dev) for _ in range(6)]
            xyz = torch.empty(Pn, 3, device=dev)
            ops.mlp_chain128_fwd(None, PE, x, bufs[0], bufs[1], acts, xyz, rows_dev=rows_dev)
            return xyz, ((None, PE, acts, (bufs[2], cond)) if save else None)
        E = torch.empty(Pn, NR_LDE, device=dev)
        ops.embed_hannw(x, band_w, cond.reshape(-1), E, PE, rows_dev=rows_dev)
        if chain:
            key = id(specs)
            bufs = self._chain_bufs.get(key)
            if bufs is None or bufs[0].device != dev:
                bufs = self._chain_bufs[key] = ops.mlp_chain_buffers(dev)
            ws = [self._w(L) for L in specs]
            ops.mlp_chain_pack([w for w, _ in ws], [b_ for _, b_ in ws], bufs[0], bufs[1])
            acts = [torch.empty(Pn, 128, device=dev) for _ in range(6)]
            xyz = torch.empty(Pn, 3, device=dev)
            ops.mlp_chain128_fwd(E, PE, x, bufs[0], bufs[1], acts, xyz, rows_dev=rows_dev)
            return xyz, ((E, PE, acts, None) if save else None)
        acts = []
        h = E
        for i in range(6):
            L = specs[i]
            Wt, bt = self._w(L)
            out = torch.empty(Pn, 128, device=dev)
            if i == 4:
                ops.linear_fwd(h, 128, Wt, bt, 128, out, ops.EPI_RELU, A1=PE, K1=NR_LDPE, rows_dev=rows_dev)
            else:
                ops.linear_fwd(h, L.Kpad, Wt, bt, 128, out, ops.EPI_RELU, rows_dev=rows_dev)
            acts.append(out)
            h = out
        Wt, bt = self._w(specs[6])
        xyz = torch.empty(Pn, 3, device=dev)
        ops.linear_fwd(h, 128, Wt, bt, 3, xyz, ops.EPI_RESIDUAL, aux=x, rows_dev=rows_dev)
        return xyz, ((E, PE, acts, None) if save else None)

    def _canonical_fwd(self, cnl: torch.Tensor, state: int, save: bool, rows_dev=None):
        Pn = cnl.shape[0]
        dev = cnl.device
        embed = self._embeds.view(self.store.param)[state]
        fold = None
        if rows_dev is not None and not ops.thin_dgrad_rows(Pn):
            raise ValueError("_canonical_fwd(rows_dev=...): the row bound exists on the thin-kernel path only (ops.thin_dgrad_rows)")
        if ops.CNL_FOLD and ops.thin_dgrad_rows(Pn):
            fkey = ("cnl_fold",) + ops._stream_key(dev)
            fb = self._chain_bufs.get(fkey)
            if fb is None:
                fb = self._chain_bufs[fkey] = torch.empty(256 * (2 * CNL_NFP + 256 + 2), device=dev)
            fw = ops.cnl_fold_views(fb, 256, CNL_NFP, 256)
            (W0, b0), (W5, b5) = self._w(self._cnl[0]), self._w(self._cnl[5])
            ops.canonical_fold_pack(W0, b0, W5, b5, embed, 256, CNL_NF, 256, fw)
            E = torch.empty(Pn, CNL_NFP, device=dev)
            CAT = torch.empty(Pn, CNL_NFP + 256, device=dev)
            ops.embed_fourier(cnl, 10, ops.zero1(dev), E, CAT, rows_dev=rows_dev)
            fold = (fw, embed)
        else:
            E = torch.empty(Pn, CNL_LDE, device=dev)
            CAT = torch.empty(Pn, CNL_CAT, device=dev)
            CAT[:, CNL_CAT - 1].zero_()
            ops.embed_fourier(cnl, 10, embed, E, CAT, rows_dev=rows_dev)
        acts, bits = [], []
        h = E
        want_bits = save and ops.thin_dgrad_rows(Pn)
        for i in range(8):
            L = self._cnl[i]
            Wt, bt = self._w(L)
            K = L.Kpad
            if fold is not None and i in (0, 5):
                Wt, bt = (fold[0][0], fold[0][1]) if i == 0 else (fold[0][2], fold[0][3])
                K = Wt.shape[1]
            rb = ops.thin_relu_bits(Pn, dev) if (want_bits and K <= 320) else None
            if i == 4:
                ops.linear_fwd(h, K, Wt, bt, 256, CAT, ops.EPI_RELU, out_col0=CNL_NFP if fold is not None else 127, relu_bits=rb,
                               rows_dev=rows_dev)
                acts.append(CAT)
                h = CAT
            else:
                out = torch.empty(Pn, 256, device=dev)
                ops.linear_fwd(h, K, Wt, bt, 256, out, ops.EPI_RELU, relu_bits=rb, rows_dev=rows_dev)
                acts.append(out)
                h = out
            bits.append(rb)
        Wt, bt = self._w(self._cnl[8])
        raw = torch.empty(Pn, 4, device=dev)
        ops.linear_fwd(h, 256, Wt, bt, 4, raw, ops.EPI_SIGMOID_RELU4, rows_dev=rows_dev)
        return raw, ((E, acts, bits, fold) if save else None)

    def _nonrigid_bwd(self, specs: List[_LayerSpec], saved, x: torch.Tensor, band_w: torch.Tensor, g_xyz: torch.Tensor, rows_dev=None):
        E, PE, acts, fold = saved
        Pn, dev = x.shape[0], x.device

        def layer_bwd(dz, X, spec, N, K, out, relu_mask, w_col0=0, bias=True, override=None):
            if override is not None:
                Wt, gW, gb = override
            else:
                Wt, _ = self._w(spec)
                gW, gb = self._w(spec, grad=True)
            ops.linear_bwd_fused(dz, X, Wt, gW, gb if bias else None, N, K, out, relu_mask, w_col0=w_col0, rows_dev=rows_dev)
            return out

        dz6 = torch.empty(Pn, 32, device=dev)
        ops.slice_pad(g_xyz, 0, 3, dz6, rows_dev=rows_dev)
        if fold is not None:
            gfold = ops.zero_(ops.fold_grad_workspace(dev))
            gw0h, db0 = gfold[:128 * 64].view(128, 64), gfold[128 * 64:]
        if (fold is not None and ops.MLP_CHAIN_BWD and Pn >= ops.MLP_CHAIN_BWD_MIN_ROWS
                and ops.get_gemm_mode() != ops.GEMM_FP32):
            Wm = [self._w(L)[0] for L in specs]
            G = [self._w(L, grad=True) for L in specs]
            im = ops.mlp_chain_bwd_images(id(specs), (0, 1, 2), dev)
            ops.mlp_chain_bwd_pack([
                (0, 0, Wm[6], 0, 3, 128, im[0][0]), (0, 1, Wm[5], 0, 128, 128, im[0][1]),
                (1, 0, Wm[4], 128, 128, NR_LDPE, im[1][0]), (1, 1, Wm[4], 0, 128, 128, im[1][1]), (1, 2, Wm[3], 0, 128, 128, im[1][2]),
                (2, 0, Wm[2], 0, 128, 128, im[2][0]), (2, 1, Wm[1], 0, 128, 128, im[2][1]), (2, 2, fold[0], 0, 128, NR_LDPE, im[2][2])])
            dPE = torch.empty(Pn, NR_LDPE, device=dev)
            dE = torch.empty(Pn, NR_LDPE, device=dev)
            dz4 = torch.empty(Pn, 128, device=dev)
            dz2 = torch.empty(Pn, 128, device=dev)
            with ops.deferred_bwd_reduce():
                ops.mlp_chain_bwd(0, dz6, [acts[5], acts[4]], im[0], [None, dz4], [G[6][0], G[5][0]], [0, 0], [G[6][1], G[5][1]],
                                  [3, 128], [128, 128], rows_dev=rows_dev)
                ops.mlp_chain_bwd(1, dz4, [PE, acts[3], acts[2]], im[1], [dPE, None, dz2], [G[4][0], G[4][0], G[3][0]], [128, 0, 0],
                                  [None, G[4][1], G[3][1]], [128, 128, 128], [NR_LDPE, 128, 128], rows_dev=rows_dev)
                ops.mlp_chain_bwd(2, dz2, [acts[1], acts[0], PE], im[2], [None, None, dE], [G[2][0], G[1][0], gw0h], [0, 0, 0],
                                  [G[2][1], G[1][1], db0], [128, 128, 128], [128, 128, NR_LDPE], rows_dev=rows_dev)
            res = g_xyz.contiguous()
            gW0, gb0 = self._w(specs[0], grad=True)
            ops.mlp_chain_unfold_grad(gw0h, db0, fold[1], 6 * band_w.numel(), gW0, gb0)
            return ops.embed_bwd_res(x, band_w, band_w.numel(), False, dE, 0, dPE, 0, res, rows_dev=rows_dev)
        with ops.deferred_bwd_reduce():
            dz = layer_bwd(dz6, acts[5], specs[6], 3, 128, torch.empty(Pn, 128, device=dev), True)
            dPE = dE = None
            for i in range(5, -1, -1):
                if i == 4:
                    dPE = layer_bwd(dz, PE, specs[4], 128, NR_LDPE, torch.empty(Pn, NR_LDPE, device=dev), False, w_col0=128, bias=False)
                    dz = layer_bwd(dz, acts[3], specs[4], 128, 128, torch.empty(Pn, 128, device=dev), True)
                elif i == 0 and fold is not None:
                    dE = layer_bwd(dz, PE, specs[0], 128, NR_LDPE, torch.empty(Pn, NR_LDPE, device=dev), False, override=(fold[0], gw0h, db0))
                elif i == 0:
                    dE = layer_bwd(dz, E, specs[0], 128, NR_LDE, torch.empty(Pn, NR_LDE, device=dev), False)
                else:
                    dz = layer_bwd(dz, acts[i - 1], specs[i], 128, 128, torch.empty(Pn, 128, device=dev), True)
        res = g_xyz.contiguous()
        if fold is not None:
            gW0, gb0 = self._w(specs[0], grad=True)
            ops.mlp_chain_unfold_grad(gw0h, db0, fold[1], 6 * band_w.numel(), gW0, gb0)
            return ops.embed_bwd_res(x, band_w, band_w.numel(), False, dE, 0, dPE, 0, res, rows_dev=rows_dev)
        return ops.embed_bwd_res(x, band_w, band_w.numel(), False, dE, 75, dPE, 0, res, rows_dev=rows_dev)

    def _canonical_bwd(self, saved, cnl: torch.Tensor, raw: torch.Tensor, g_raw: torch.Tensor, state: int, rows_dev=None):
        E, acts, bits, fold = saved
        rd = rows_dev
        CAT = acts[4]
        Pn, dev = cnl.shape[0], cnl.device
        dz8 = torch.empty(Pn, 32, device=dev)
        ops.rgbsigma_grad(g_raw.contiguous(), raw, dz8, rows_dev=rd)
        Wt, _ = self._w(self._cnl[8])
        gW, gb = self._w(self._cnl[8], grad=True)
        ops.linear_wgrad(dz8, acts[7], gW, gb, 4, 256, rows_dev=rd)
        dz = torch.empty(Pn, 256, device=dev)
        ops.linear_dgrad(dz8, Wt, 32, 256, dz, mask_src=acts[7], mask_bits=bits[7], rows_dev=rd)
        dCAT = dE = None
        tmp_b = {}
        if fold is not None:
            gws = ops.zero_(ops.cnl_fold_grad_workspace(dev, 256, CNL_NFP, 256))
            gfold = ops.cnl_fold_views(gws, 256, CNL_NFP, 256)
        with ops.deferred_bwd_reduce():
            for i in range(7, -1, -1):
                L = self._cnl[i]
                Wt, _ = self._w(L)
                gW, gb = self._w(L, grad=True)
                if i == 5 and fold is not None:
                    W5f = fold[0][2]
                    ops.linear_wgrad(dz, CAT, gfold[2], gfold[3], 256, CNL_NFP + 256, rows_dev=rd)
                    nxt = torch.empty(Pn, 256, device=dev)
                    dCAT = torch.empty(Pn, CNL_NFP, device=dev)
                    ops.linear_dgrad(dz, W5f, 256, CNL_NFP, dCAT, thin=True, rows_dev=rd)
                    ops.linear_dgrad(dz, W5f, 256, 256, nxt, mask_src=CAT, w_col0=CNL_NFP, mask_col0=CNL_NFP, mask_bits=bits[4], rows_dev=rd)
                    dz = nxt
                elif i == 0 and fold is not None:
                    ops.linear_wgrad(dz, E, gfold[0], gfold[1], 256, CNL_NFP, rows_dev=rd)
                    dE = torch.empty(Pn, CNL_NFP, device=dev)
                    ops.linear_dgrad(dz, fold[0][0], 256, CNL_NFP, dE, thin=True, rows_dev=rd)
                elif i == 5:
                    tmp_b[5] = ops.zeros(L.Npad, dev)
                    ops.linear_wgrad(dz, CAT, gW, tmp_b[5], 256, CNL_CAT, rows_dev=rd)
                    nxt = torch.empty(Pn, 256, device=dev)
                    if ops.thin_dgrad_rows(Pn):
                        dCAT = torch.empty(Pn, 64, device=dev)
                        ops.linear_dgrad(dz, Wt, 256, 64, dCAT, thin=True, rows_dev=rd)
                        ops.linear_dgrad(dz, Wt, 256, 256, nxt, mask_src=CAT, w_col0=127, mask_col0=127, mask_bits=bits[4], rows_dev=rd)
                    else:
                        dCAT = torch.empty(Pn, CNL_CAT, device=dev)
                        ops.linear_dgrad(dz, Wt, 256, CNL_CAT, dCAT, rows_dev=rd)
                        ops.slice_mask(dCAT, 127, CAT, 127, 256, nxt, rows_dev=rd)
                    dz = nxt
                elif i == 0:
                    tmp_b[0] = ops.zeros(L.Npad, dev)
                    ops.linear_wgrad(dz, E, gW, tmp_b[0], 256, CNL_LDE, rows_dev=rd)
                    dE = torch.empty(Pn, CNL_LDE, device=dev)
                    ops.linear_dgrad(dz, Wt, 256, CNL_LDE, dE, rows_dev=rd)
                else:
                    inp = acts[i - 1]
                    ops.linear_wgrad(dz, inp, gW, gb, 256, 256, rows_dev=rd)
                    nxt = torch.empty(Pn, 256, device=dev)
                    ops.linear_dgrad(dz, Wt, 256, 256, nxt, mask_src=inp, mask_bits=bits[i - 1], rows_dev=rd)
                    dz = nxt
        g_embed = self._embeds.view(self.store.grad)[state]
        if fold is not None:
            (W0, _), (W5, _) = self._w(self._cnl[0]), self._w(self._cnl[5])
            (gW0, gb0), (gW5, gb5) = self._w(self._cnl[0], grad=True), self._w(self._cnl[5], grad=True)
            ops.canonical_fold_unfold(gfold, W0, W5, fold[1], 256, CNL_NF, 256, gW0, gb0, gW5, gb5, g_embed)
        else:
            for i in (0, 5):
                Wt, _ = self._w(self._cnl[i])
                _, gb = self._w(self._cnl[i], grad=True)
                gb += tmp_b[i]
                g_embed.addmv_(Wt[:256, 63:127].t(), tmp_b[i][:256])
        g_cnl = torch.empty(Pn, 3, device=dev)
        ops.embed_bwd(cnl, None, 10, True, dE, 0, dCAT, 0, g_cnl, False, rows_dev=rd)
        return g_cnl

    def frame_prologue(self, dst_Rs, dst_Ts, cnl_gtfms, motion_weights_priors, dst_posevec=None, iter_val=1e7, **kwargs):
        cfg = self.cfg
        K = cfg.total_bones
        iter_v = float(torch.as_tensor(iter_val).reshape(-1)[0])
        time = float(kwargs["time"])
        is_train = bool(kwargs["is_train"])
        flow = time > 0.005 and is_train
        nr_kick = cfg.non_rigid_motion_mlp.kick_in_iter

        def cond_of(pv):
            return torch.zeros_like(pv) * pv if iter_v < nr_kick else pv

        if flow and dst_Rs.is_cuda and not (dst_Rs.requires_grad or dst_Ts.requires_grad or dst_posevec.requires_grad):
            nR, nT, nP = dst_Rs.numel(), dst_Ts.numel(), dst_posevec.numel()
            pad4 = lambda n: (2 * n + 3) // 4 * 4
            buf = torch.empty(pad4(nR) + pad4(nT) + pad4(nP), device=dst_Rs.device)
            Rs = buf[:2 * nR].view((2,) + tuple(dst_Rs.shape))
            Ts = buf[pad4(nR):pad4(nR) + 2 * nT].view((2,) + tuple(dst_Ts.shape))
            pv = buf[pad4(nR) + pad4(nT):pad4(nR) + pad4(nT) + 2 * nP].view(2, nP)
            c = lambda t_: t_.detach().float().contiguous()
            ops.copy_or_zero_n([Rs[0], Rs[1], Ts[0], Ts[1], pv[0], pv[1]],
                               [c(dst_Rs), c(kwargs["dst_Rs_prev"]), c(dst_Ts), c(kwargs["dst_Ts_prev"]), c(dst_posevec).reshape(-1),
                                c(kwargs["dst_posevec_prev"]).reshape(-1)])
        elif flow:
            Rs = torch.stack([dst_Rs, kwargs["dst_Rs_prev"]], 0)
            Ts = torch.stack([dst_Ts, kwargs["dst_Ts_prev"]], 0)
            pv = torch.stack([dst_posevec.reshape(-1), kwargs["dst_posevec_prev"].reshape(-1)], 0)
        else:
            Rs, Ts, pv = dst_Rs[None], dst_Ts[None], dst_posevec.reshape(1, -1)
        if iter_v >= cfg.pose_decoder.get("kick_in_iter", 0):
            Rs, Ts = self._pose_refine(Rs, Ts, pv)
        Rb_, Tb_, Rf_, Tf_ = self._motion_basis(Rs, Ts, cnl_gtfms)
        vol = self._motion_weight_volume(motion_weights_priors)
        if self.split_decoder_backward and torch.is_grad_enabled() and vol.requires_grad:
            self._fwd_stream = torch.cuda.current_stream(vol.device) if vol.is_cuda else None
            leaf = vol.detach().requires_grad_(True)
            self._pending_vol = (vol, leaf)
            vol = leaf
        Rb, Tb, Rf, Tf = ops.unbind_frames_many(Rb_, Tb_, Rf_, Tf_)
        vol, vol_cl = ops.volume_pair(vol, K)
        pro = {"flow": flow, "state": select_state(time, self.transitions_times), "R_b": Rb[0], "T_b": Tb[0],
               "R_f": Rf[0], "T_f": Tf[0], "band_w": self._band_weights(iter_v, dst_Rs.device),
               "cond": cond_of(dst_posevec).contiguous(), "vol": vol, "vol_cl": vol_cl}
        if flow:
            pro.update(R_fp=Rf[1], T_fp=Tf[1], cond_prev=cond_of(kwargs["dst_posevec_prev"]).contiguous())
        return pro

    def forward(self, rays, dst_Rs=None, dst_Ts=None, cnl_gtfms=None, motion_weights_priors=None, dst_posevec=None, near=None,
                far=None, iter_val=1e7, t_rand=None, prologue=None, with_cycle: bool = True, static_cycle: bool = False,
                live_rays: bool = False, **kwargs):
        return ops.guarded_forward(self, rays.device, lambda: self._forward(
            rays, dst_Rs, dst_Ts, cnl_gtfms, motion_weights_priors, dst_posevec, near, far, iter_val, t_rand, prologue, with_cycle,
            static_cycle, live_rays, **kwargs))

    def _forward(self, rays, dst_Rs=None, dst_Ts=None, cnl_gtfms=None, motion_weights_priors=None, dst_posevec=None, near=None,
                 far=None, iter_val=1e7, t_rand=None, prologue=None, with_cycle: bool = True, static_cycle: bool = False,
                 live_rays: bool = False, **kwargs):
        cfg = self.cfg
        dev = rays.device
        K = cfg.total_bones
        pro = prologue if prologue is not None else self.frame_prologue(
            dst_Rs, dst_Ts, cnl_gtfms, motion_weights_priors, dst_posevec=dst_posevec, iter_val=iter_val, **kwargs)
        flow, state, band_w, cond, vol, vol_cl = pro["flow"], pro["state"], pro["band_w"], pro["cond"], pro["vol"], pro["vol_cl"]
        R_b, T_b, R_f, T_f = pro["R_b"], pro["T_b"], pro["R_f"], pro["T_f"]
        if flow:
            R_fp, T_fp, cond_prev = pro["R_fp"], pro["T_fp"], pro["cond_prev"]
        bmin = kwargs["cnl_bbox_min_xyz"].contiguous()
        bscale = kwargs["cnl_bbox_scale_xyz"].contiguous()

        rays_o = rays[0].reshape(-1, 3).float().contiguous()
        rays_d = rays[1].reshape(-1, 3).float().contiguous()
        B = rays_o.shape[0]
        N = cfg.N_samples
        if t_rand is None and cfg.perturb > 0.0:
            t_rand = torch.rand(B, N, device=dev)
        outs: Dict[str, List[torch.Tensor]] = {}
        chunk = int(cfg.chunk)
        live_rays = bool(live_rays and self.stage == 3 and B <= chunk and torch.is_grad_enabled() and ops.thin_dgrad_rows(B * N))
        for c0 in range(0, B, chunk):
            sl = slice(c0, min(B, c0 + chunk))
            tr = None if t_rand is None else t_rand[sl].contiguous()
            grad = torch.is_grad_enabled()
            live = rows_live = None
            if live_rays:
                z, pts, x_skel, mask = ops.human_sample_warp_ad(vol, R_b, T_b, rays_o[sl], rays_d[sl], near[sl].contiguous(),
                                                                far[sl].contiguous(), N, bmin, bscale, tr, K)
                live = ops.select_live_rays(mask.detach().view(-1, N))
                rows_live = live.rows
                x_c = ops.gather_rays(x_skel.reshape(-1, 3), live)
                mask_c = ops.gather_rays(mask.detach().reshape(-1, 1), live).view(-1)
                pts_c = ops.gather_rays(pts.detach().reshape(-1, 3), live)
                cnl = _NonRigidFn.apply(self._token, self, "nr", x_c, cond, band_w, rows_live)
                n_use = 1 + int(flow) + int(with_cycle)
                cnl_uses = list(ops.fanout(cnl, n_use))
                raw = ops.scatter_rays(_CanonicalFn.apply(self._token, self, cnl_uses.pop(), state, rows_live), live)
            elif grad:
                z, pts, x_skel, mask = ops.human_sample_warp_ad(vol, R_b, T_b, rays_o[sl], rays_d[sl], near[sl].contiguous(),
                                                                far[sl].contiguous(), N, bmin, bscale, tr, K)
                cnl = _NonRigidFn.apply(self._token, self, "nr", x_skel, cond, band_w, None)
                n_use = 1 + int(flow) + int(with_cycle)
                cnl_uses = list(ops.fanout(cnl, n_use))
                raw = _CanonicalFn.apply(self._token, self, cnl_uses.pop(), state)
            else:
                z, pts, x_skel, mask = ops.human_sample_warp(rays_o[sl], rays_d[sl], near[sl].contiguous(), far[sl].contiguous(),
                                                             N, R_b, T_b, vol, bmin, bscale, tr, K)
                cnl, _ = self._nonrigid_fwd(self._nr, x_skel, cond, band_w, save=False)
                cnl_uses = [cnl, cnl, cnl]
                raw, _ = self._canonical_fwd(cnl, state, save=False)
            b = z.shape[0]
            if self.stage == 2:
                rgb_map, acc_map, weights, depth_map = ops.raw2outputs(raw.view(b, N, 4), z, rays_d[sl], mask.view(b, N),
                                                                       kwargs["bgcolor"].to(dev))
                ret = {"rgb": rgb_map, "alpha": acc_map, "depth": depth_map, "weights": weights}
            else:
                ret = {"human_rgb": raw[:, :3].reshape(b, N, 3), "human_density": raw[:, 3].reshape(b, N),
                       "human_rgbsigma": raw.view(b, N, 4), "newsmpl_pts": pts, "pts_mask": mask.view(b, N)}

            def fwd_branch(c_pts, Rf_, Tf_, cond_, rows_dev=None):
                if grad:
                    d_ = ops.lbs_forward_ad(c_pts, vol_cl, Rf_, Tf_, bmin, bscale, K, rows_dev=rows_dev)
                    return _NonRigidFn.apply(self._token, self, "nrf", d_, cond_, band_w, rows_dev)
                d_ = ops.lbs_forward(c_pts, Rf_, Tf_, vol_cl, bmin, bscale, K, rows_dev=rows_dev)
                return self._nonrigid_fwd(self._nrf, d_, cond_, band_w, save=False, rows_dev=rows_dev)[0]

            if flow and live is not None:
                ret["deform_pts_prev_final"] = ops.scatter_rays(fwd_branch(cnl_uses.pop(), R_fp, T_fp, cond_prev, rows_dev=rows_live),
                                                                live).view(b, N, 3)
            elif flow:
                ret["deform_pts_prev_final"] = fwd_branch(cnl_uses.pop(), R_fp, T_fp, cond_prev).view(b, N, 3)
            cyc_mask, cyc_pts = (mask_c, pts_c) if live is not None else (mask, pts)
            if with_cycle and static_cycle:
                if B > chunk:
# ... 61 lines not shown
```

hosnerf_amd/ops.py:

```python
from __future__ import annotations

import os
import threading

import math
from typing import Optional, Tuple

import numpy as np
import torch

from . import _lib
from ._lib import call, ptr

EPS = 1.1920929e-07

EPI_NONE, EPI_RELU, EPI_DENSITY, EPI_RGB, EPI_NERF_HEAD, EPI_SIGMOID_RELU4, EPI_RESIDUAL = 0, 1, 2, 3, 4, 5, 6


def round_up(x: int, m: int) -> int:
    return (x + m - 1) // m * m


class KernelEvents:

# ... 84 lines not shown
LIVE_RAYS = True
_CNL_FOLD_WS = {}
_ZERO1 = {}


def zero1(device) -> torch.Tensor:
    key = str(torch.device(device))
    if key not in _ZERO1:
        _ZERO1[key] = torch.zeros(1, device=device)
    return _ZERO1[key]


def _table(ptrs, ctype=None):
    import ctypes
    ctype = ctypes.c_void_p if ctype is None else ctype
    return (ctype * len(ptrs))(*ptrs)


def clear_last_error() -> int:
    return int(_lib.load().hos_clear_last_error())


def copy_or_zero_n(dsts, srcs=None):
    import ctypes
    for i0 in range(0, len(dsts), 8):
        d = dsts[i0:i0 + 8]
        sr = [None] * len(d) if srcs is None else srcs[i0:i0 + 8]
        for a, b in zip(d, sr):
            if b is not None and b.numel() != a.numel():
                raise _lib.HosLibraryError("copy_or_zero_n: size mismatch")
        call("hos_copy_or_zero_n", len(d), _table([ptr(t) for t in d]), _table([ptr(t) for t in sr]),
             _table([t.numel() for t in d], ctypes.c_longlong))


def zeros_many(shapes, device, dtype=torch.float32):
    sizes = [(int(np.prod(sh)) + 3) // 4 * 4 for sh in shapes]
    buf = torch.empty(sum(sizes), device=device, dtype=dtype)
    copy_or_zero_n([buf])
    out, o = [], 0
    for sh, n in zip(shapes, sizes):
        out.append(buf[o:o + int(np.prod(sh))].view(sh))
        o += n
    return out


def zeros(shape, device):
    shape = (shape,) if isinstance(shape, int) else tuple(shape)
    return zeros_many([shape], device)[0]


def zero_(t: torch.Tensor):
    copy_or_zero_n([t])
    return t


def add_n(ts):
    import ctypes
    out = torch.empty_like(ts[0])
    call("hos_add_n", len(ts), _table([ptr(t.contiguous()) for t in ts]), ts[0].numel(), ptr(out))
    return out


class _Fanout(torch.autograd.Function):

    @staticmethod
    def forward(ctx, x, n):
        ctx.set_materialize_grads(False)
        return tuple(x.view_as(x) for _ in range(n))

    @staticmethod
    def backward(ctx, *gs):
        gs = [g.contiguous() for g in gs if g is not None]
        if not gs:
            return None, None
        return (gs[0] if len(gs) == 1 else add_n(gs)), None


def fanout(x: torch.Tensor, n: int):
    return _Fanout.apply(x, n) if (n > 1 and x.requires_grad and torch.is_grad_enabled()) else (x,) * n


def canonical_fold_pack(W0, b0, W5, b5, embed, n_out, nf, nh, out):
    call("hos_canonical_fold_pack", ptr(W0), W0.stride(0), ptr(b0), ptr(W5), W5.stride(0), ptr(b5), ptr(embed), n_out, nf, embed.numel(), nh,
         ptr(out[0]), ptr(out[1]), ptr(out[2]), ptr(out[3]))


def canonical_fold_unfold(grads, W0, W5, embed, n_out, nf, nh, gW0, gb0, gW5, gb5, g_embed):
    call("hos_canonical_fold_unfold", ptr(grads[0]), ptr(grads[1]), ptr(grads[2]), ptr(grads[3]), ptr(W0), W0.stride(0), ptr(W5), W5.stride(0),
         ptr(embed), n_out, nf, embed.numel(), nh, ptr(gW0), ptr(gb0), ptr(gW5), ptr(gb5), ptr(g_embed))


def cnl_fold_views(buf: torch.Tensor, n_out: int, nfp: int, nh: int):
    o1 = n_out * nfp
    o2 = o1 + n_out
    o3 = o2 + n_out * (nfp + nh)
    return buf[:o1].view(n_out, nfp), buf[o1:o2], buf[o2:o3].view(n_out, nfp + nh), buf[o3:o3 + n_out]


def cnl_fold_grad_workspace(device, n_out: int, nfp: int, nh: int) -> torch.Tensor:
    key = _stream_key(device) + (n_out, nfp, nh)
    if key not in _CNL_FOLD_WS:
        _CNL_FOLD_WS[key] = torch.empty(n_out * (2 * nfp + nh + 2), device=device)
    return _CNL_FOLD_WS[key]


def thin_dgrad_rows(M: int) -> bool:
    return bool(M >= 16384 and _lib.load().hos_get_gemm_mode() == GEMM_BF16X3)


def thin_relu_bits(M: int, device) -> torch.Tensor:
    return torch.empty(((M + 31) // 32) * 512, dtype=torch.int16, device=device)


def linear_dgrad(dY: torch.Tensor, W: torch.Tensor, Npad: int, K: int, out: torch.Tensor,
                 mask_src: Optional[torch.Tensor] = None, accumulate: bool = False, w_col0: int = 0, mask_col0: int = 0,
                 thin: bool = False, mask_bits: Optional[torch.Tensor] = None, rows_dev: Optional[torch.Tensor] = None):
    M = dY.shape[0]
    wptr = ptr(W) + 4 * w_col0
    mptr = None if mask_src is None else ptr(mask_src) + 4 * mask_col0
    if mask_bits is not None and K > 256:
        raise _lib.HosLibraryError("mask_bits cover one thin launch (K <= 256 columns)")
    if (not accumulate and Npad <= 256 and Npad % 4 == 0 and (K > 128 or thin) and thin_dgrad_rows(M)):
        for k0 in range(0, K, 256):
            kc = min(256, K - k0)
            _timed(f"thin_dgrad[M={M},N={kc},K={Npad}]", 2.0 * M * kc * Npad, lambda: call(
                "hos_thin_linear_dgrad", ptr(dY), dY.stride(0), wptr + 4 * k0, W.stride(0), Npad,
                None if mptr is None else mptr + 4 * k0, 0 if mask_src is None else mask_src.stride(0), ptr(mask_bits, torch.int16),
                ptr(out) + 4 * k0, out.stride(0), M, kc, ptr(rows_dev, torch.int32)))
        return out
    if rows_dev is not None:
        raise _lib.HosLibraryError("rows_dev: this layer does not run on the thin kernel (check ops.thin_dgrad_rows first)")
    if mask_bits is not None and mask_src is None:
        raise _lib.HosLibraryError("mask_bits: this layer does not run on the thin kernel (check ops.thin_dgrad_rows first)")
    _timed(f"gemm_dgrad[M={M},N={K},K={Npad}]", 2.0 * M * K * Npad, lambda: call(
        "hos_linear_dgrad", ptr(dY), dY.stride(0), wptr, W.stride(0), Npad, mptr,
        0 if mask_src is None else mask_src.stride(0), ptr(out), out.stride(0), M, K, int(accumulate)))
    return out


def linear_wgrad(dY: torch.Tensor, X: torch.Tensor, dW: torch.Tensor, db: Optional[torch.Tensor], N: int, K: int,
                 w_col0: int = 0, splits: int = 0, rows_dev: Optional[torch.Tensor] = None):
    M = dY.shape[0]
    if 128 < N <= 256 and M >= 16384 and _lib.load().hos_get_gemm_mode() == GEMM_BF16X3:
        for k0 in range(0, K, 256):
            kc = min(256, K - k0)
            ws = _bwd_workspace(dY.device, M, N, kc, False)
            _timed(f"wgrad_tr[M={N},N={kc},K={M}]", 2.0 * M * N * kc, lambda: call(
                "hos_linear_wgrad_tr", ptr(dY), dY.stride(0), ptr(X) + 4 * k0, X.stride(0), ptr(dW) + 4 * (w_col0 + k0), dW.stride(0),
                ptr(db) if k0 == 0 else None, M, N, kc, ptr(ws), ws.numel(), ptr(rows_dev, torch.int32)))
        return
    _timed(f"gemm_wgrad[M={N},N={K},K={M}]", 2.0 * M * N * K, lambda: call(
        "hos_linear_wgrad", ptr(dY), dY.stride(0), ptr(X), X.stride(0), ptr(dW) + 4 * w_col0, dW.stride(0),
        ptr(db), M, N, K, splits, ptr(rows_dev, torch.int32)))


def linear_bwd_fused(dY: torch.Tensor, X: torch.Tensor, W: torch.Tensor, dW: torch.Tensor, db: Optional[torch.Tensor], N: int,
                     K: int, out: Optional[torch.Tensor], relu_mask: bool, w_col0: int = 0, rows_dev: Optional[torch.Tensor] = None):
    M = dY.shape[0]
    ws = _bwd_workspace(dY.device, M, N, K, True)
    _timed(f"mlp_bwd_fused[M={M},N={N},K={K}]", 4.0 * M * N * K, lambda: call(
        "hos_linear_bwd_fused", ptr(dY), dY.stride(0), ptr(X), X.stride(0), ptr(W) + 4 * w_col0, W.stride(0),
        ptr(out), 0 if out is None else out.stride(0), ptr(dW) + 4 * w_col0, dW.stride(0), ptr(db), M, N, K, int(relu_mask),
        ptr(ws), ws.numel(), ptr(rows_dev, torch.int32)))
    return out


_BWD_WS = {}
_BWD_DEFER = {"on": False, "offset": 0}


def _stream_key(device):
    d = torch.device(device)
    return (str(d), torch.cuda.current_stream(d).cuda_stream if d.type == "cuda" else 0)


def _bwd_workspace(device, M: int = 0, N: int = 0, K: int = 0, fused: bool = False, need: Optional[int] = None) -> torch.Tensor:
    key = _stream_key(device)
    if not _BWD_DEFER["on"]:
        if key not in _BWD_WS:
            _BWD_WS[key] = torch.empty(256 * (256 * 256 + 256), device=device)
        return _BWD_WS[key][:256 * (256 * 256 + 256)]
    if need is None:
        need = int(_lib.load().hos_mlp_bwd_ws_floats(M, N, K, int(fused)))
    need = max((need + 3) // 4 * 4, 4)
    ws = _BWD_WS.get(key)
    if ws is None or ws.numel() < max(need, BWD_DEFER_WS_FLOATS):
        _BWD_WS[key] = ws = torch.empty(max(need, BWD_DEFER_WS_FLOATS), device=device)
    if _BWD_DEFER["offset"] + need > ws.numel():
        call("hos_mlp_bwd_flush")
        _BWD_DEFER["offset"] = 0
    off = _BWD_DEFER["offset"]
    _BWD_DEFER["offset"] = off + need
    return ws[off:off + need]


BWD_DEFER_WS_FLOATS = 160 * 1024 * 1024


class deferred_bwd_reduce:

    def __enter__(self):
        self.nested = _BWD_DEFER["on"]
        if not self.nested:
            _BWD_DEFER["on"], _BWD_DEFER["offset"] = True, 0
            _lib.check(_lib.load().hos_mlp_bwd_defer(1), "hos_mlp_bwd_defer")
        return self

    def __exit__(self, *exc):
        if not self.nested:
            _BWD_DEFER["on"] = False
            _lib.check(_lib.load().hos_mlp_bwd_defer(0), "hos_mlp_bwd_defer")
            call("hos_mlp_bwd_flush")
        return False


MLP_CHAIN = True
MLP_CHAIN_MIN_ROWS = 4096
MLP_CHAIN_FOLD = True
_FOLD_WS = {}


def fold_grad_workspace(device) -> torch.Tensor:
    key = _stream_key(device)
    if key not in _FOLD_WS:
        _FOLD_WS[key] = torch.empty(128 * 64 + 128, device=device)
    return _FOLD_WS[key]
MLP_CHAIN_BWD = True
MLP_CHAIN_BWD_MIN_ROWS = 16384
_CB_IMAGES = {}
_CB_IMAGES_MAX = 16


def _int_array(vals):
    import ctypes
    return (ctypes.c_int * len(vals))(*[int(v) for v in vals])


def mlp_chain_bwd_images(key, cfgs, device):
    lib = _lib.load()
    k = (key, tuple(cfgs)) + _stream_key(device)
    bufs = _CB_IMAGES.get(k)
    if bufs is None:
        while len(_CB_IMAGES) >= _CB_IMAGES_MAX:
            _CB_IMAGES.pop(next(iter(_CB_IMAGES)))
        bufs = _CB_IMAGES[k] = [[torch.empty(int(lib.hos_mlp_chain_bwd_image_bytes(c, s)) // 2, dtype=torch.int16, device=device)
                                 for s in range(int(lib.hos_mlp_chain_bwd_steps(c)))] for c in cfgs]
    return bufs


def mlp_chain_bwd_pack(jobs):
    import ctypes
    for i in range(0, len(jobs), 8):
        js = jobs[i:i + 8]
        Wp = (ctypes.c_void_p * len(js))(*[ptr(j[2]) + 4 * j[3] for j in js])
        call("hos_mlp_chain_bwd_pack", len(js), _int_array([j[0] for j in js]), _int_array([j[1] for j in js]), Wp,
             _int_array([j[2].stride(0) for j in js]), _int_array([j[4] for j in js]), _int_array([j[5] for j in js]),
             (ctypes.c_void_p * len(js))(*[ptr(j[6], torch.int16) for j in js]))


def mlp_chain_bwd(cfg, dZ, X, images, dXout, dW, w_col0, db, N, K, rows_dev=None):
    import ctypes
    M = dZ.shape[0]
    S = len(X)
    need = int(_lib.load().hos_mlp_chain_bwd_ws_floats(cfg, M))
    ws = _bwd_workspace(dZ.device, need=need)
    flop = sum(4.0 * M * n * k for n, k in zip(N, K))
    _timed(f"mlp_chain_bwd{cfg}[M={M}]", flop, lambda: call(
        "hos_mlp_chain_bwd", cfg, ptr(dZ), dZ.stride(0), M, ptr(rows_dev, torch.int32), _ptr_array(list(X)), _int_array([x.stride(0) for x in X]),
        (ctypes.c_void_p * S)(*[ptr(im, torch.int16) for im in images]), _ptr_array(list(dXout)),
        _int_array([0 if o is None else o.stride(0) for o in dXout]),
        (ctypes.c_void_p * S)(*[ptr(g) + 4 * c for g, c in zip(dW, w_col0)]), _int_array([g.stride(0) for g in dW]),
        _ptr_array(list(db)), _int_array(N), _int_array(K), ptr(ws), ws.numel()))


def mlp_chain_buffers(device):
    lib = _lib.load()
    return (torch.empty(int(lib.hos_mlp_chain_weight_bytes()) // 2, dtype=torch.int16, device=device),
            torch.empty(int(lib.hos_mlp_chain_aux_floats()), device=device))


def mlp_chain_pack(weights, biases, planes, aux):
    import ctypes
    ldw = (ctypes.c_int * 7)(*[int(w.stride(0)) for w in weights])
    call("hos_mlp_chain_pack", _ptr_array(list(weights)), ldw, _ptr_array(list(biases)), ptr(planes, torch.int16), ptr(aux))


def mlp_chain_pack_fold(weights, biases, cond, nfeat, planes, aux, w0h):
    import ctypes
    ldw = (ctypes.c_int * 7)(*[int(w.stride(0)) for w in weights])
    call("hos_mlp_chain_pack_fold", _ptr_array(list(weights)), ldw, _ptr_array(list(biases)), ptr(cond), cond.numel(), nfeat,
         ptr(planes, torch.int16), ptr(aux), ptr(w0h))


def mlp_chain_unfold_grad(gw0h, db, cond, nfeat, gW0, gb0):
    call("hos_mlp_chain_unfold_grad", ptr(gw0h), ptr(db), ptr(cond), cond.numel(), nfeat, ptr(gW0), gW0.stride(0), ptr(gb0))


def mlp_chain128_fwd(E, PE, x, planes, aux, acts, xyz, rows_dev=None):
    P = x.shape[0]
    flop = 101120 if E is not None else 101120 - 128 * 64
    _timed(f"mlp_chain128{'' if E is not None else 'f'}[M={P}]", 2.0 * P * flop, lambda: call(
        "hos_mlp_chain128_fwd", ptr(E), 0 if E is None else E.stride(0), ptr(PE), PE.stride(0), ptr(x), ptr(planes, torch.int16), ptr(aux),
        _ptr_array(list(acts)), acts[0].stride(0), ptr(xyz), P, ptr(rows_dev, torch.int32)))


_RANGE_FLAG = {}
# ... 1400 lines not shown
```

include/hosrender.h:

```cpp
#ifndef HOSRENDER_H
#define HOSRENDER_H

#include <stdint.h>

#ifdef __cplusplus
extern "C" {
#endif

#define HOS_OK 0
#define HOS_E_ARG (-1)
#define HOS_E_ALIGN (-2)
#define HOS_E_SHAPE (-3)
#define HOS_E_NODEVICE (-4)

typedef void* hos_stream_t;

#define HOS_ABI_VERSION 101

int hos_version(void);
int hos_device_count(void);
const char* hos_error_string(int code);


#define HOS_GEMM_MODE_FP32 0
#define HOS_GEMM_MODE_BF16X3 1
int hos_set_gemm_mode(int mode);
int hos_set_thread_gemm_mode(int mode);
int hos_get_gemm_mode(void);

int hos_set_range_flag(unsigned int* flag);

#define HOS_EPI_NONE 0
#define HOS_EPI_RELU 1
#define HOS_EPI_DENSITY 2
#define HOS_EPI_RGB 3
#define HOS_EPI_NERF_HEAD 4
#define HOS_EPI_SIGMOID_RELU4 5
#define HOS_EPI_RESIDUAL 6

int hos_linear_fwd(const float* A0, int lda0, int K0, const float* A1, int lda1, int K1,
                   const float* W, int ldw, const float* bias, float* C, int ldc,
                   int M, int N, int epilogue, float* aux, int aux_col, float p0, float p1,
                   const int32_t* rows_dev, hos_stream_t stream);

int hos_linear_fwd_splitk(const float* A, int lda, const float* W, int ldw, float* C, int ldc, int M, int N, int K,
                          hos_stream_t stream);
long long hos_linear_fwd_splitk_ws_floats(int M, int N, int K);
int hos_linear_fwd_splitk_det(const float* A, int lda, const float* W, int ldw, const float* bias, int relu, float* C, int ldc,
                              int M, int N, int K, float* ws, long long ws_floats, hos_stream_t stream);

int hos_linear_dgrad(const float* dY, int lddy, const float* W, int ldw, int Npad,
                     const float* Xact, int ldx, float* dX, int lddx, int M, int K,
                     int accumulate, hos_stream_t stream);

int hos_linear_wgrad(const float* dY, int lddy, const float* X, int ldx, float* dW, int ldw,
                     float* db, int M, int N, int K, int splits, const int32_t* rows_dev, hos_stream_t stream);

int hos_linear_bwd_fused(const float* dY, int lddy, const float* X, int ldx, const float* W, int ldw,
                         float* dX, int lddx, float* dW, int lddw, float* db, int M, int N, int K,
                         int relu_mask, float* ws, int64_t ws_floats, const int32_t* rows_dev,
                         hos_stream_t stream);

int hos_mlp_bwd_defer(int on);
int hos_mlp_bwd_flush(hos_stream_t stream);
long long hos_mlp_bwd_ws_floats(int M, int N, int K, int fused);

int hos_linear_wgrad_tr(const float* dY, int lddy, const float* X, int ldx, float* dW, int lddw, float* db,
                        int M, int N, int K, float* ws, int64_t ws_floats, const int32_t* rows_dev, hos_stream_t stream);

int hos_thin_linear_fwd(const float* X, int ldx, const float* W, int ldw, const float* bias, float* Y, int ldy,
                        int M, int N, int K, int epilogue, void* relu_bits, const int32_t* rows_dev, hos_stream_t stream);
int hos_thin_linear_dgrad(const float* dY, int lddy, const float* W, int ldw, int Npad, const float* mask, int ldmask,
                          const void* mask_bits, float* dX, int lddx, int M, int K, const int32_t* rows_dev, hos_stream_t stream);

int hos_canonical_fold_pack(const float* W0, int ld0, const float* b0, const float* W5, int ld5, const float* b5,
                            const float* embed, int n_out, int nf, int ne, int nh,
                            float* W0f, float* b0f, float* W5f, float* b5f, hos_stream_t stream);
int hos_canonical_fold_unfold(const float* gW0f, const float* db0, const float* gW5f, const float* db5,
                              const float* W0, int ld0, const float* W5, int ld5, const float* embed,
                              int n_out, int nf, int ne, int nh,
                              float* gW0, float* gb0, float* gW5, float* gb5, float* g_embed, hos_stream_t stream);


int hos_split_planes(const float* src, int lds, int R, int C, int dtype, void* out, int ldo,
                     void* outT, int ldt, hos_stream_t stream);

int hos_split_planes_t_batch(int n, const float* const* src, const int* lds, const int* R, const int* C, void* const* outT,
                             const int* ldt, hos_stream_t stream);

int hos_split_planes2(const float* src, int lds, int R, int C, void* p16, int ld16, void* pb, int ldb,
                      hos_stream_t stream);

int hos_linearp_fwd(const void* A, int lda, int K0, const void* A1, int lda1, int K1, const void* W, int ldw,
                    const float* bias, int M, int N, int relu, void* Y, int ldy, void* Yb, int ldyb, void* relu_bits,
                    float* C, int ldc, int epilogue, float* aux, int aux_col, float p0, hos_stream_t stream);

int hos_planes_rowdot(const void* A, int lda, int K, const float* w, const float* bias, float p0, int softplus, int64_t M,
                      float* out, hos_stream_t stream);

int hos_linearp_fwd_b(const void* A, int lda, int K0, const void* A1, int lda1, int K1, const void* W, int ldw,
                      const float* bias, int M, int N, int relu, void* Y, int ldy, void* relu_bits,
                      float* C, int ldc, int epilogue, float* aux, int aux_col, float p0, hos_stream_t stream);
int hos_planes_rowdot_b(const void* A, int lda, int K, const float* w, const float* bias, float p0, int softplus, int64_t M,
                        float* out, hos_stream_t stream);

int hos_linearp_dgrad(const void* dZ, int lddz, const void* WT, int ldwt, int Npad, const void* mask, int ldmask,
                      const void* mask_bits, int M, int K, void* dX, int lddx, hos_stream_t stream);

int hos_linearp_wgrad(const void* dZ, int lddz, const void* X, int ldx, int x_col0, float* dW, int ldw, float* db,
                      int M, int N, int K, int splits, float* ws, long long ws_floats, hos_stream_t stream);


int hos_camera_rays(const float* Kinv9, const float* R9, const float* T3, int H, int W, float* rays_o, float* rays_d,
                    float* viewdirs, float* radii, hos_stream_t stream);

int hos_rays_aabb(const float* rays_o, float* rays_d, int64_t n, const float* bounds6, float* near, float* far,
                  unsigned char* mask, hos_stream_t stream);

int hos_frame_rays_compact(const float* Kinv9, const float* R9, const float* T3, const float* bounds6, int H, int W,
                           float* rays_o, float* rays_d, float* near, float* far, int32_t* pix, int32_t* slot,
                           int32_t* count, int32_t* ws, hos_stream_t stream);

int hos_frame_paint(const int32_t* slot, const float* rgb, int count, const float* bg01, int H, int W, float* out_f32,
                    unsigned char* out_u8, hos_stream_t stream);


int hos_raybank_index(const unsigned char* keep, int N, int H, int W, int32_t* pix, int64_t cap, int32_t* counts,
                      int64_t* offsets, int32_t* ws, hos_stream_t stream);

int hos_raybank_gather(const float* cams, const float* times, const unsigned char* images, const int32_t* pix,
                       const int64_t* offsets, const int32_t* counts, const int32_t* img_id, const int32_t* rank,
                       int64_t B, int N, int H, int W, int64_t cap, float* rays_o, float* rays_d, float* viewdirs,
                       float* radii, float* times_out, float* target, hos_stream_t stream);

int hos_raybank_frame(const float* cam16, float time, int H, int W, int64_t start, int64_t n, const unsigned char* image,
                      float* rays_o, float* rays_d, float* viewdirs, float* radii, float* times_out, float* target,
                      hos_stream_t stream);


int hos_deconv3d_col2im(const float* ycol, const float* bias, int D, int Cout, float leaky_slope, int leaky,
                        float* out, hos_stream_t stream);

int hos_deconv3d_im2col(const float* dpre, int D, int Cout, float* dycol, hos_stream_t stream);
int hos_bias_lrelu(float* y, const float* bias, long long M, int N, float leaky_slope, int leaky, hos_stream_t stream);
int hos_shard_interleave(const float* parts, int world, int M, int cs, float* out, hos_stream_t stream);

int hos_deconv3d_dpre(const float* g, const float* out, long long R, int C, float leaky_slope, int leaky, float* dpre, float* db,
                      hos_stream_t stream);
int hos_outer_accum(const float* x, int ldx, const float* dy, int lddy, float* gW, int ldw, int M, int K, int N,
                    hos_stream_t stream);
long long hos_gemv_ws_floats(int K, int N);
int hos_gemv_rowvec(const float* x, const float* W, int ldw, int K, int N, const float* bias, int bias_mod,
                    float leaky_slope, int leaky, float* ws, float* y, hos_stream_t stream);


int hos_resample(const float* sdist_prev, const float* w_prev, int n_prev, int B, int S,
                 float dilation, float anneal, const float* train_frac_dev, float anneal_slope,
                 float resample_padding, const float* u_base, const float* jitter, float jitter_scale,
                 float near_, float far_, float* sdist, float* tdist, int32_t* bin_idx,
                 hos_stream_t stream);

int hos_encode_ipe(const float* tdist, const float* rays_o, const float* rays_d, const float* radii,
                   const float* basis, const float* embed, int B, int S, float* X, int ldx,
                   hos_stream_t stream);

int hos_encode_ipe_planes(const float* tdist, const float* rays_o, const float* rays_d, const float* radii,
                          const float* basis, const float* embed, int B, int S, void* p16, void* pb, int ld,
                          hos_stream_t stream);

int hos_encode_viewdirs(const float* viewdirs, int B, int S, float* Xv, int ldx, int col0,
                        hos_stream_t stream);

int hos_alpha_weights_fwd(const float* density, const float* tdist, const float* dirs, int B, int S,
                          int opaque_background, float* weights, hos_stream_t stream);
int hos_alpha_weights_bwd(const float* g_weights, const float* density, const float* tdist,
                          const float* dirs, int B, int S, int opaque_background, float* g_density,
                          hos_stream_t stream);

int hos_volrender_fwd(const float* rgbs, const float* weights, int B, int S, float bg, float* rgb,
                      hos_stream_t stream);
int hos_volrender_bwd(const float* g_rgb, const float* rgbs, const float* weights, int B, int S,
                      float bg, float* g_rgbs, float* g_weights, hos_stream_t stream);
int hos_volrender_maps_fwd(const float* rgbs, const float* weights, const float* tdist, int B, int S, float bg,
                           float* rgb, float* acc, float* depth, float* depth_median, hos_stream_t stream);

int hos_interlevel_fwd(const float* c, const float* w, const float* cp, const float* wp, int B,
                       int Sc, int Sp, float* loss_ray, int32_t* idx_lo, int32_t* idx_hi,
                       hos_stream_t stream);
int hos_interlevel_bwd(const float* c, const float* w, const float* cp, const float* wp, int B,
                       int Sc, int Sp, float scale, float* g_wp, hos_stream_t stream);
int hos_distortion_fwd(const float* t, const float* w, int B, int S, float* loss_ray,
                       hos_stream_t stream);
int hos_distortion_bwd(const float* t, const float* w, int B, int S, float scale, float* g_w,
                       hos_stream_t stream);

int hos_head_grad(const float* g_density, const float* density, const float* g_rgb, const float* rgb,
                  int P, float rgb_padding, float* dz_density, int ld_dd, int col_dd,
                  float* dz_rgb, int ld_dr, hos_stream_t stream);


int hos_human_sample_warp(const float* rays_o, const float* rays_d, const float* near_, const float* far_,
                          const float* t_vals, const float* t_rand, const float* R, const float* T,
                          const float* vol, int V, const float* bbox_min, const float* bbox_scale,
                          int B, int N, int K, float* z_vals, float* pts, float* x_skel, float* mask,
                          hos_stream_t stream);

int hos_lbs_forward(const float* cnl_pts, const float* R_fwd, const float* T_fwd, const float* vol_cl,
                    int V, int CL, const float* bbox_min, const float* bbox_scale, int64_t P, int K,
                    float* x_deform, const int32_t* rows_dev, hos_stream_t stream);

int hos_embed_hannw(const float* x, const float* band_w, int num_freqs, const float* cond, int cond_size,
                    int64_t P, float* E, int lde, float* PE, int ldpe, const int32_t* rows_dev, hos_stream_t stream);

int hos_embed_fourier(const float* x, int num_freqs, const float* state, int state_size, int64_t P,
                      float* E, int lde, float* E2, int lde2, const int32_t* rows_dev, hos_stream_t stream);

int hos_human_sample_warp_bwd(const float* pts, const float* R, const float* T, const float* vol, int V,
                              const float* bbox_min, const float* bbox_scale, int64_t P, int K,
                              const float* g_x_skel, const float* g_mask, float* g_vol, float* g_R, float* g_T,
                              float* scratch, const float* fwd_x_skel, const float* fwd_mask, hos_stream_t stream);
int hos_lbs_forward_bwd(const float* cnl_pts, const float* R_fwd, const float* T_fwd, const float* vol_cl,
                        int V, int CL, const float* bbox_min, const float* bbox_scale, int64_t P, int K,
                        const float* g_x_deform, float* g_cnl, float* g_vol_cl, float* g_R, float* g_T,
                        const int32_t* rows_dev, hos_stream_t stream);
int hos_embed_bwd(const float* x, const float* band_w, int num_freqs, int identity, const float* dA, int lda,
                  int colA, const float* dB, int ldb, int colB, int64_t P, float* g_x, int accumulate,
// ... 189 lines not shown
```

Measured before the change: 141,100.

## Fuse canonical MLP 256->4 head into last hidden layer forward and backward

The 4-wide output head of the canonical MLP is computed inside the epilogue of layer 7's thin forward GEMM: per-tile partial dot products go to shared memory and are reduced one tile later, so the separate head GEMM launch and the re-read of the 256-wide activation are removed. In backward, the 256-wide gradient for layer 7 is no longer materialised. The wgrad and dgrad kernels rebuild it on the fly from the 4-wide head gradient, the head weights and the ReLU bits. This saves a launch plus a full Pn x 256 write and read, at the cost of more shared memory, extra epilogue arithmetic and recomputing the head gradient in two kernels.

```diff
diff --git a/hosnerf_amd/csrc/hos_gemm_common.h b/hosnerf_amd/csrc/hos_gemm_common.h
--- a/hosnerf_amd/csrc/hos_gemm_common.h
+++ b/hosnerf_amd/csrc/hos_gemm_common.h
@@ -49,6 +49,24 @@
 }
 __device__ __forceinline__ float quad_xor2(float x) {
     return __int_as_float(__builtin_amdgcn_mov_dpp(__float_as_int(x), 0x4E, 0xF, 0xF, true));
+}
+
+__device__ __forceinline__ int th_head_word(int wave, int lane) { return (lane >> 3) * 64 + 4 * (lane & 7) + (wave & 3) + 32 * ((wave >> 2) & 1); }
+__device__ __forceinline__ float4 head_row(float x, int i) {
+    const int xi = __float_as_int(x);
+    return make_float4(__int_as_float(__builtin_amdgcn_readlane(xi, 4 * i + 0)), __int_as_float(__builtin_amdgcn_readlane(xi, 4 * i + 1)),
+                       __int_as_float(__builtin_amdgcn_readlane(xi, 4 * i + 2)), __int_as_float(__builtin_amdgcn_readlane(xi, 4 * i + 3)));
+}
+__device__ __forceinline__ float4 th_head_dz(const float4& g, const float4 (&hw)[4], uint32_t bits, int i) {
+    float v[4];
+    const float w[4][4] = {{hw[0].x, hw[0].y, hw[0].z, hw[0].w}, {hw[1].x, hw[1].y, hw[1].z, hw[1].w},
+                           {hw[2].x, hw[2].y, hw[2].z, hw[2].w}, {hw[3].x, hw[3].y, hw[3].z, hw[3].w}};
+#pragma unroll
+    for (int k = 0; k < 4; ++k) {
+        const float s = fmaf(g.w, w[3][k], fmaf(g.z, w[2][k], fmaf(g.y, w[1][k], g.x * w[0][k])));
+        v[k] = __uint_as_float(__float_as_uint(s) & (uint32_t)__builtin_amdgcn_sbfe((int)bits, 15 - (4 * i + k), 1));
+    }
+    return make_float4(v[0], v[1], v[2], v[3]);
 }
 
 template <int MODE>
diff --git a/hosnerf_amd/csrc/hos_mlpbwd.hip b/hosnerf_amd/csrc/hos_mlpbwd.hip
--- a/hosnerf_amd/csrc/hos_mlpbwd.hip
+++ b/hosnerf_amd/csrc/hos_mlpbwd.hip
@@ -21,6 +21,8 @@
     float* ws;
     int ws_dw;
     const int* m_dev;
+    const float* hW; int ldhw;
+    const uint16_t* hbits;
 };
 
 constexpr int mb_rows(bool dg) { return dg ? 64 : 32; }
@@ -281,7 +283,7 @@
     }
 }
 
-template <int KT>
+template <int KT, bool HEAD = false>
 __global__ __launch_bounds__(MB_NT, 1) void wgrad_tr_fast_kernel(MlpBwdArgs a) {
     constexpr int NT = 8, N_ = NT * 32, K_ = KT * 32, R = 32;
     constexpr int PZ = N_ * 2 + 32, PX = K_ * 2 + 32;
@@ -307,15 +309,30 @@
     const int nrb = (a.m_dev ? min(a.M, *a.m_dev) : a.M) / R;
     const int G = gridDim.x;
     float4 rzA[ZU], rxA[XU], rzB[ZU], rxB[XU];
+    uint32_t hbA = 0, hbB = 0;
+    static_assert(!HEAD || ZU == 4, "th_head_word: rows wave + 8 i, i < 4");
+    float* const hwl = reinterpret_cast<float*>(Xl + X_PLANE);
+    const int hword = th_head_word(wave, lane);
+    if constexpr (HEAD) {
+        if (t < 256) {
+#pragma unroll
+            for (int j = 0; j < 4; ++j) hwl[j * 256 + t] = a.hW[(size_t)j * a.ldhw + t];
+        }
+        __syncthreads();
+    }
     float4 bsum = make_float4(0.f, 0.f, 0.f, 0.f);
-    auto gload = [&](float4 (&rz)[ZU], float4 (&rx)[XU], int rb) {
+    auto gload = [&](float4 (&rz)[ZU], float4 (&rx)[XU], uint32_t& hb, int rb) {
         rb = rb < nrb ? rb : nrb - 1;
         const float* zb = a.dZ + (size_t)rb * R * a.lddz;
         const float* xb = a.X + (size_t)rb * R * a.ldx;
 #pragma unroll
         for (int i = 0; i < ZU; ++i) {
             const int u = t + MB_NT * i, row = u / (N_ / 4), c4 = u % (N_ / 4);
-            rz[i] = ldg4(zb + (size_t)row * a.lddz + c4 * 4);
+            if constexpr (!HEAD) rz[i] = ldg4(zb + (size_t)row * a.lddz + c4 * 4);
+        }
+        if constexpr (HEAD) {
+            rz[0].x = zb[(size_t)(wave + 8 * ((lane >> 2) & 3)) * a.lddz + (lane & 3)];
+            hb = a.hbits[(size_t)rb * MB_NT + hword];
         }
 #pragma unroll
         for (int i = 0; i < XU; ++i) {
@@ -323,13 +340,20 @@
             rx[i] = ldg4(xb + (size_t)row * a.ldx + c4 * 4);
         }
     };
-    auto sstore = [&](const float4 (&rz)[ZU], const float4 (&rx)[XU]) {
+    auto sstore = [&](const float4 (&rz)[ZU], const float4 (&rx)[XU], const uint32_t hb) {
+        float4 hw[HEAD ? 4 : 1];
+        if constexpr (HEAD) {
+#pragma unroll
+            for (int j = 0; j < 4; ++j) hw[j] = *reinterpret_cast<const float4*>(hwl + j * 256 + 4 * lane);
+        }
 #pragma unroll
         for (int i = 0; i < ZU; ++i) {
             const int u = t + MB_NT * i, row = u / (N_ / 4), c4 = u % (N_ / 4);
-            bsum.x += rz[i].x; bsum.y += rz[i].y; bsum.z += rz[i].z; bsum.w += rz[i].w;
+            float4 z = rz[i];
+            if constexpr (HEAD) z = th_head_dz(head_row(rz[0].x, i), hw, hb, i);
+            bsum.x += z.x; bsum.y += z.y; bsum.z += z.z; bsum.w += z.w;
             bf16x4 h, l;
-            split4(rz[i], h, l);
+            split4(z, h, l);
             *reinterpret_cast<bf16x4*>(Zh + row * PZ + c4 * 8) = h;
             *reinterpret_cast<bf16x4*>(Zl + row * PZ + c4 * 8) = l;
         }
@@ -367,28 +391,28 @@
         }
     };
 #define WG_BAR() asm volatile("s_waitcnt lgkmcnt(0)\n\ts_barrier" ::: "memory")
-    auto step = [&](float4 (&rz)[ZU], float4 (&rx)[XU], const int rb) {
-        sstore(rz, rx);
+    auto step = [&](float4 (&rz)[ZU], float4 (&rx)[XU], uint32_t& hb, const int rb) {
+        sstore(rz, rx, hb);
         WG_BAR();
-        gload(rz, rx, rb + 2 * G);
+        gload(rz, rx, hb, rb + 2 * G);
         compute();
         WG_BAR();
     };
     int rb = blockIdx.x;
     if (rb < nrb) {
-        gload(rzA, rxA, rb);
-        gload(rzB, rxB, rb + G);
-        step(rzA, rxA, rb);
+        gload(rzA, rxA, hbA, rb);
+        gload(rzB, rxB, hbB, rb + G);
+        step(rzA, rxA, hbA, rb);
         rb += G;
         if (rb < nrb) {
-            step(rzB, rxB, rb);
+            step(rzB, rxB, hbB, rb);
             rb += G;
             while (rb + G < nrb) {
-                step(rzA, rxA, rb);
-                step(rzB, rxB, rb + G);
+                step(rzA, rxA, hbA, rb);
+                step(rzB, rxB, hbB, rb + G);
                 rb += 2 * G;
             }
-            if (rb < nrb) step(rzA, rxA, rb);
+            if (rb < nrb) step(rzA, rxA, hbA, rb);
         }
     }
 #undef WG_BAR
@@ -529,21 +553,21 @@
     return hos_launch_status();
 }
 
-template <int KT>
+template <int KT, bool HEAD = false>
 int launch_wgrad_fast(MlpBwdArgs a, size_t ws_floats, hipStream_t stream) {
     constexpr int N_ = 256, K_ = KT * 32, R = 32, nk = N_ * K_;
-    constexpr size_t smem = 2 * (size_t)R * (N_ * 2 + 32) + 2 * (size_t)R * (K_ * 2 + 32);
+    constexpr size_t smem = 2 * (size_t)R * (N_ * 2 + 32) + 2 * (size_t)R * (K_ * 2 + 32) + (HEAD ? 4096 : 0);
     const int nrb = a.M / R;
     const int grid = nrb < 256 ? nrb : 256;
     if (a.M % R != 0 || a.N != N_ || a.K != K_ || a.ws == nullptr || grid < 32 ||
         ws_floats < (size_t)grid * (nk + N_) || (((uintptr_t)a.ws) & 15u)) return -1;
     static bool attr_set = false;
     if (!attr_set) {
-        hipError_t e = hipFuncSetAttribute(reinterpret_cast<const void*>(&wgrad_tr_fast_kernel<KT>), hipFuncAttributeMaxDynamicSharedMemorySize, (int)smem);
+        hipError_t e = hipFuncSetAttribute(reinterpret_cast<const void*>(&wgrad_tr_fast_kernel<KT, HEAD>), hipFuncAttributeMaxDynamicSharedMemorySize, (int)smem);
         if (e != hipSuccess) return (int)e;
         attr_set = true;
     }
-    hipLaunchKernelGGL((wgrad_tr_fast_kernel<KT>), dim3(grid), dim3(MB_NT), smem, stream, a);
+    hipLaunchKernelGGL((wgrad_tr_fast_kernel<KT, HEAD>), dim3(grid), dim3(MB_NT), smem, stream, a);
     if (g_defer) {
         if (g_batch.count == MB_BATCH) { const int rc = flush_reduce_batch(stream); if (rc != 0) return rc; }
         ReduceJob& J = g_batch.j[g_batch.count];
@@ -970,6 +994,18 @@
     return launch_mb<8, 8, false>(a, (size_t)ws_floats, s);
 }
 
+extern "C" int hos_linear_wgrad_tr_head(const float* dZh, int lddzh, const float* Wh, int ldwh, const void* head_bits,
+                                        const float* X, int ldx, float* dW, int lddw, float* db, int M, float* ws, int64_t ws_floats,
+                                        const int32_t* rows_dev, hos_stream_t stream) {
+    if (!dZh || !Wh || !head_bits || !X || !dW || !ws || M <= 0 || ws_floats <= 0) return HOS_E_ARG;
+    if ((lddzh & 3) || (ldwh & 3) || (ldx & 3) || lddzh < 4 || ldwh < 256 || ldx < 256) return HOS_E_ALIGN;
+    if ((((uintptr_t)dZh | (uintptr_t)Wh | (uintptr_t)X) & 15u) || ((uintptr_t)head_bits & 1u)) return HOS_E_ALIGN;
+    MlpBwdArgs a{dZh, lddzh, X, ldx, nullptr, 0, nullptr, 0, dW, lddw, db, M, 256, 256, 0, ws, 0, rows_dev,
+                 Wh, ldwh, static_cast<const uint16_t*>(head_bits)};
+    const int rc = launch_wgrad_fast<8, true>(a, (size_t)ws_floats, static_cast<hipStream_t>(stream));
+    return rc == -1 ? HOS_E_SHAPE : rc;
+}
+
 extern "C" int hos_mlp_bwd_defer(int on) { g_defer = on != 0; return 0; }
 
 extern "C" int hos_mlp_bwd_flush(hos_stream_t stream) { return flush_reduce_batch(static_cast<hipStream_t>(stream)); }
diff --git a/hosnerf_amd/csrc/hos_thin.hip b/hosnerf_amd/csrc/hos_thin.hip
--- a/hosnerf_amd/csrc/hos_thin.hip
+++ b/hosnerf_amd/csrc/hos_thin.hip
@@ -34,6 +34,10 @@
     unsigned int* range_flag;
     uint16_t* bits;
     const int* m_dev;
+    const float* hW; int ldhw;
+    const float* hb;
+    float* raw;
+    const uint16_t* hbits;
 };
 
 __device__ __forceinline__ int th_live_tiles(const ThinArgs& a) { return (a.m_dev ? min(a.M, *a.m_dev) : a.M) / 32; }
@@ -243,7 +247,13 @@
     }
 }
 
-template <int KS, bool BITS>
+constexpr int TH_HEAD_PART = 16 * 32 * 16;
+template <int N>
+__device__ __forceinline__ float row_ror_add(float x) {
+    return x + __int_as_float(__builtin_amdgcn_update_dpp(0, __float_as_int(x), 0x120 + N, 0xF, 0xF, false));
+}
+
+template <int KS, bool BITS, bool HEAD = false>
 __global__ __launch_bounds__(TH_NT, 1) void thin_fwd_fast_kernel(const ThinArgs a) {
     typedef _Float16 E;
     typedef typename V8<E>::t e8;
@@ -255,7 +265,7 @@
     constexpr int P = KD * 2 + TH_PAD_FWD;
     constexpr int PLANE = R * P, BUF = 2 * PLANE;
     constexpr int AU = R * (KD / 4) / TH_NT;
-    constexpr bool PF2 = KS <= TH_PF2_MAXKS;
+    constexpr bool PF2 = KS <= TH_PF2_MAXKS && !HEAD;
     constexpr int PFD = PF2 ? 3 : 2;
     static_assert(AU >= 1 && R * (KD / 4) % TH_NT == 0, "tile does not divide over 512 threads");
 
@@ -279,6 +289,26 @@
     const int q4 = l31 & 3, colb = col0 + (l31 & ~3);
     const float4 bias4 = a.bias != nullptr ? ld4(a.bias + colb) : make_float4(0.f, 0.f, 0.f, 0.f);
     const bool relu = a.epi == HOS_EPI_RELU;
+    char* const part0 = smem_th + 2 * BUF;
+    float* const hwl = reinterpret_cast<float*>(part0 + 2 * TH_HEAD_PART);
+    float hbj = 0.f;
+    if constexpr (HEAD) {
+        if (t < 256) {
+#pragma unroll
+            for (int j = 0; j < 4; ++j) hwl[j * 256 + t] = a.hW[(size_t)j * a.ldhw + t];
+        }
+        if (a.hb != nullptr) hbj = a.hb[lane & 3];
+    }
+    auto head_out = [&](const int ptile, const int pb) {
+        if (lane < 16) {
+            const char* p = part0 + pb * TH_HEAD_PART + (4 * wave + (lane >> 2)) * 16 + (lane & 3) * 4;
+            float s = *reinterpret_cast<const float*>(p);
+#pragma unroll
+            for (int k = 1; k < 16; ++k) s += *reinterpret_cast<const float*>(p + k * 512);
+            s += hbj;
+            a.raw[(size_t)ptile * 128 + 16 * wave + lane] = (lane & 3) < 3 ? sigmoid_f(s) : fmaxf(s, 0.f);
+        }
+    };
 
     const int G = gridDim.x;
     float4 ra[AU], rb[PF2 ? AU : 1];
@@ -313,7 +343,8 @@
     if constexpr (PF2) gload(rb, tile + 2 * G);
     __syncthreads();
     bool big = false;
-    auto body = [&](float4 (&rcur)[AU], const int tile, const int b, const bool more) {
+    auto body = [&](float4 (&rcur)[AU], const int tile, const int b, const bool more, const bool hasprev = true) {
+        if constexpr (HEAD) { if (hasprev) head_out(tile - G, b ^ 1); }
         const char* hi = buf0 + b * BUF + l31 * P + lhi * 16;
         f32x16 acc;
 #pragma unroll
@@ -352,6 +383,19 @@
             if (relu) { v[0] = fmaxf(v[0], 0.f); v[1] = fmaxf(v[1], 0.f); v[2] = fmaxf(v[2], 0.f); v[3] = fmaxf(v[3], 0.f); }
             big |= (fmaxf(fmaxf(fabsf(v[0]), fabsf(v[1])), fmaxf(fabsf(v[2]), fabsf(v[3]))) > HOS_RANGE_LIMIT) | (pre != pre);
             *reinterpret_cast<float4*>(crow + (size_t)(8 * g) * a.ldc) = make_float4(v[0], v[1], v[2], v[3]);
+            if constexpr (HEAD) {
+                float hp[4];
+#pragma unroll
+                for (int j = 0; j < 4; ++j) {
+                    const float4 hv = *reinterpret_cast<const float4*>(hwl + j * 256 + colb);
+                    float s = fmaf(v[3], hv.w, fmaf(v[2], hv.z, fmaf(v[1], hv.y, v[0] * hv.x)));
+                    s = row_ror_add<4>(s);
+                    hp[j] = row_ror_add<8>(s);
+                }
+                if ((lane & 12) == 0)
+                    *reinterpret_cast<float4*>(part0 + b * TH_HEAD_PART + (2 * wave + ((lane >> 4) & 1)) * 512 + (q4 + 4 * lhi + 8 * g) * 16) =
+                        make_float4(hp[0], hp[1], hp[2], hp[3]);
+            }
         }
         if constexpr (BITS) {
             const uint32_t odd = (uint32_t)__builtin_amdgcn_mov_dpp((int)rbits, 0xB1, 0xF, 0xF, true);
@@ -361,7 +405,7 @@
     };
     int b = 0;
     if constexpr (PF2) {
-        body(ra, tile, b, tile + G < ntiles);
+        body(ra, tile, b, tile + G < ntiles, false);
         tile += G; b ^= 1;
         if (tile < ntiles) {
             body(rb, tile, b, tile + G < ntiles);
@@ -371,17 +415,18 @@
                 body(rb, tile + G, b ^ 1, tile + 2 * G < ntiles);
                 tile += 2 * G;
             }
-            if (tile < ntiles) body(ra, tile, b, false);
+            if (tile < ntiles) { body(ra, tile, b, false); tile += G; b ^= 1; }
         }
     } else {
-        body(ra, tile, b, tile + G < ntiles);
+        body(ra, tile, b, tile + G < ntiles, false);
         tile += G; b ^= 1;
         for (; tile < ntiles; tile += G, b ^= 1) body(ra, tile, b, tile + G < ntiles);
     }
+    if constexpr (HEAD) head_out(tile - G, b ^ 1);
     if (a.range_flag != nullptr && __builtin_amdgcn_ballot_w64(big) != 0 && lane == 0) atomicOr(a.range_flag, 1u);
 }
 
-template <bool MASK>
+template <bool MASK, bool HEAD = false>
 __global__ __launch_bounds__(TH_NT, 1) void thin_dgrad_fast_kernel(const ThinArgs a) {
     typedef __bf16 E;
     typedef typename V8<E>::t e8;
@@ -414,24 +459,43 @@
     const int G = gridDim.x;
     float4 ra[AU], rb[AU];
     uint32_t ba = 0, bb = 0, bits_staged = 0;
+    static_assert(!HEAD || AU == 4, "th_head_word: rows wave + 8 i, i < 4");
+    float* const hwl = reinterpret_cast<float*>(smem_th + 2 * BUF);
+    const int hword = th_head_word(wave, lane);
+    if constexpr (HEAD) {
+        if (t < 256) {
+#pragma unroll
+            for (int j = 0; j < 4; ++j) hwl[j * 256 + t] = a.hW[(size_t)j * a.ldhw + t];
+        }
+        __syncthreads();
+    }
     auto gload = [&](float4 (&r)[AU], uint32_t& rbits, int tile) {
         tile = tile < ntiles ? tile : ntiles - 1;
         const float* base = a.A + (size_t)tile * R * a.lda;
 #pragma unroll
         for (int i = 0; i < AU; ++i) {
             const int u = t + TH_NT * i, row = u / (KD / 4), c4 = u % (KD / 4);
-            r[i] = ld4(base + (size_t)row * a.lda + c4 * 4);
-        }
+            if constexpr (!HEAD) r[i] = ld4(base + (size_t)row * a.lda + c4 * 4);
+        }
+        if constexpr (HEAD) r[0].x = base[(size_t)(wave + 8 * ((lane >> 2) & 3)) * a.lda + (lane & 3)];
         if constexpr (MASK) rbits = a.bits[(size_t)tile * TH_NT + t];
+        if constexpr (HEAD) rbits = (MASK ? rbits : 0u) | ((uint32_t)a.hbits[(size_t)tile * TH_NT + hword] << 16);
     };
     auto sstore = [&](const float4 (&r)[AU], const uint32_t rbits, int b) {
         char* const hi = buf0 + b * BUF;
         char* const lo = hi + PLANE;
+        float4 hw[HEAD ? 4 : 1];
+        if constexpr (HEAD) {
+#pragma unroll
+            for (int j = 0; j < 4; ++j) hw[j] = *reinterpret_cast<const float4*>(hwl + j * 256 + 4 * lane);
+        }
 #pragma unroll
         for (int i = 0; i < AU; ++i) {
             const int u = t + TH_NT * i, row = u / (KD / 4), c4 = u % (KD / 4);
             e4 h, l;
-            const float xs[4] = {r[i].x, r[i].y, r[i].z, r[i].w};
+            float4 x = r[i];
+            if constexpr (HEAD) x = th_head_dz(head_row(r[0].x, i), hw, rbits >> 16, i);
+            const float xs[4] = {x.x, x.y, x.z, x.w};
 #pragma unroll
             for (int q = 0; q < 4; ++q) { E hh, ll; split_pair<E>(xs[q], hh, ll); h[q] = hh; l[q] = ll; }
             *reinterpret_cast<e4*>(hi + row * P + c4 * 8) = h;
@@ -507,35 +571,35 @@
     else run(std::false_type{});
 }
 
-template <bool MASK>
+template <bool MASK, bool HEAD = false>
 int launch_thin_dgrad_fast(const ThinArgs& a, hipStream_t stream) {
-    constexpr size_t smem = 2 * 2 * (size_t)32 * (16 * 32 + th_pad<true>());
+    constexpr size_t smem = 2 * 2 * (size_t)32 * (16 * 32 + th_pad<true>()) + (HEAD ? 4096 : 0);
     static bool attr_set = false;
     if (!attr_set) {
-        hipError_t e = hipFuncSetAttribute(reinterpret_cast<const void*>(&thin_dgrad_fast_kernel<MASK>),
+        hipError_t e = hipFuncSetAttribute(reinterpret_cast<const void*>(&thin_dgrad_fast_kernel<MASK, HEAD>),
                                            hipFuncAttributeMaxDynamicSharedMemorySize, (int)smem);
         if (e != hipSuccess) return (int)e;
         attr_set = true;
     }
     const int ntiles = a.M / 32;
     const int grid = ntiles < 256 ? ntiles : 256;
-    hipLaunchKernelGGL((thin_dgrad_fast_kernel<MASK>), dim3(grid), dim3(TH_NT), smem, stream, a);
+    hipLaunchKernelGGL((thin_dgrad_fast_kernel<MASK, HEAD>), dim3(grid), dim3(TH_NT), smem, stream, a);
     return hos_launch_status();
 }
 
-template <int KS, bool BITS>
+template <int KS, bool BITS, bool HEAD = false>
 int launch_thin_fast(const ThinArgs& a, hipStream_t stream) {
-    constexpr size_t smem = 2 * 2 * (size_t)32 * (KS * 32 + TH_PAD_FWD);
+    constexpr size_t smem = 2 * 2 * (size_t)32 * (KS * 32 + TH_PAD_FWD) + (HEAD ? 2 * TH_HEAD_PART + 4096 : 0);
     static bool attr_set = false;
     if (!attr_set) {
-        hipError_t e = hipFuncSetAttribute(reinterpret_cast<const void*>(&thin_fwd_fast_kernel<KS, BITS>),
+        hipError_t e = hipFuncSetAttribute(reinterpret_cast<const void*>(&thin_fwd_fast_kernel<KS, BITS, HEAD>),
                                            hipFuncAttributeMaxDynamicSharedMemorySize, (int)smem);
         if (e != hipSuccess) return (int)e;
         attr_set = true;
     }
     const int ntiles = a.M / 32;
     const int grid = ntiles < 256 ? ntiles : 256;
-    hipLaunchKernelGGL((thin_fwd_fast_kernel<KS, BITS>), dim3(grid), dim3(TH_NT), smem, stream, a);
+    hipLaunchKernelGGL((thin_fwd_fast_kernel<KS, BITS, HEAD>), dim3(grid), dim3(TH_NT), smem, stream, a);
     return hos_launch_status();
 }
 
@@ -677,3 +741,31 @@
     }
     return Npad <= 128 ? launch_thin<8, true>(a, s) : launch_thin<16, true>(a, s);
 }
+
+extern "C" int hos_thin_linear_fwd_head(const float* X, int ldx, const float* W, int ldw, const float* bias, float* Y, int ldy,
+                                        const float* Wh, int ldwh, const float* bh, float* raw, int M, void* relu_bits,
+                                        const int32_t* rows_dev, hos_stream_t stream) {
+    if (!X || !W || !Y || !Wh || !raw || M <= 0) return HOS_E_ARG;
+    if (M & 31) return HOS_E_SHAPE;
+    if ((ldx & 3) || (ldw & 3) || (ldy & 3) || (ldwh & 3) || ldx < 256 || ldw < 256 || ldy < 256 || ldwh < 256) return HOS_E_ALIGN;
+    if ((((uintptr_t)X | (uintptr_t)W | (uintptr_t)Y | (uintptr_t)Wh | (uintptr_t)bias) & 15u) || ((uintptr_t)relu_bits & 3u) ||
+        (((uintptr_t)raw | (uintptr_t)bh) & 3u)) return HOS_E_ALIGN;
+    ThinArgs a{X, ldx, W, ldw, bias, Y, ldy, M, 256, 256, HOS_EPI_RELU, nullptr, 0, hos_range_flag_ptr(), static_cast<uint16_t*>(relu_bits),
+               rows_dev, Wh, ldwh, bh, raw, nullptr};
+    hipStream_t s = static_cast<hipStream_t>(stream);
+    return relu_bits ? launch_thin_fast<16, true, true>(a, s) : launch_thin_fast<16, false, true>(a, s);
+}
+
+extern "C" int hos_thin_linear_dgrad_head(const float* dZh, int lddzh, const float* Wh, int ldwh, const void* head_bits,
+                                          const float* W, int ldw, const void* mask_bits, float* dX, int lddx, int M,
+                                          const int32_t* rows_dev, hos_stream_t stream) {
+    if (!dZh || !Wh || !head_bits || !W || !dX || M <= 0) return HOS_E_ARG;
+    if (M & 31) return HOS_E_SHAPE;
+    if ((lddzh & 3) || (ldwh & 3) || (lddx & 3) || lddzh < 4 || ldwh < 256 || ldw < 256 || lddx < 256) return HOS_E_ALIGN;
+    if ((((uintptr_t)dZh | (uintptr_t)Wh | (uintptr_t)dX) & 15u) || ((uintptr_t)W & 3u) || (((uintptr_t)head_bits | (uintptr_t)mask_bits) & 1u))
+        return HOS_E_ALIGN;
+    ThinArgs a{dZh, lddzh, W, ldw, nullptr, dX, lddx, M, 256, 256, 0, nullptr, 0, nullptr, static_cast<uint16_t*>(const_cast<void*>(mask_bits)),
+               rows_dev, Wh, ldwh, nullptr, nullptr, static_cast<const uint16_t*>(head_bits)};
+    hipStream_t s = static_cast<hipStream_t>(stream);
+    return mask_bits ? launch_thin_dgrad_fast<true, true>(a, s) : launch_thin_dgrad_fast<false, true>(a, s);
+}
diff --git a/hosnerf_amd/human_nerf.py b/hosnerf_amd/human_nerf.py
--- a/hosnerf_amd/human_nerf.py
+++ b/hosnerf_amd/human_nerf.py
@@ -502,6 +502,8 @@
         acts, bits = [], []
         h = E
         want_bits = save and ops.thin_dgrad_rows(Pn)
+        raw = torch.empty(Pn, 4, device=dev)
+        head = ops.cnl_head_rows(Pn)
         for i in range(8):
             L = self._cnl[i]
             Wt, bt = self._w(L)
@@ -510,7 +512,13 @@
                 Wt, bt = (fold[0][0], fold[0][1]) if i == 0 else (fold[0][2], fold[0][3])
                 K = Wt.shape[1]
             rb = ops.thin_relu_bits(Pn, dev) if (want_bits and K <= 320) else None
-            if i == 4:
+            if i == 7 and head:
+                Wh, bh = self._w(self._cnl[8])
+                out = torch.empty(Pn, 256, device=dev)
+                ops.linear_fwd_head(h, Wt, bt, out, Wh, bh, raw, relu_bits=rb, rows_dev=rows_dev)
+                acts.append(out)
+                h = out
+            elif i == 4:
                 ops.linear_fwd(h, K, Wt, bt, 256, CAT, ops.EPI_RELU, out_col0=CNL_NFP if fold is not None else 127, relu_bits=rb,
                                rows_dev=rows_dev)
                 acts.append(CAT)
@@ -521,9 +529,9 @@
                 acts.append(out)
                 h = out
             bits.append(rb)
-        Wt, bt = self._w(self._cnl[8])
-        raw = torch.empty(Pn, 4, device=dev)
-        ops.linear_fwd(h, 256, Wt, bt, 4, raw, ops.EPI_SIGMOID_RELU4, rows_dev=rows_dev)
+        if not head:
+            Wt, bt = self._w(self._cnl[8])
+            ops.linear_fwd(h, 256, Wt, bt, 4, raw, ops.EPI_SIGMOID_RELU4, rows_dev=rows_dev)
         return raw, ((E, acts, bits, fold) if save else None)
 
     def _nonrigid_bwd(self, specs: List[_LayerSpec], saved, x: torch.Tensor, band_w: torch.Tensor, g_xyz: torch.Tensor, rows_dev=None):
@@ -598,8 +606,12 @@
         Wt, _ = self._w(self._cnl[8])
         gW, gb = self._w(self._cnl[8], grad=True)
         ops.linear_wgrad(dz8, acts[7], gW, gb, 4, 256, rows_dev=rd)
-        dz = torch.empty(Pn, 256, device=dev)
-        ops.linear_dgrad(dz8, Wt, 32, 256, dz, mask_src=acts[7], mask_bits=bits[7], rows_dev=rd)
+        head = ops.cnl_head_rows(Pn) and bits[7] is not None
+        Wh = Wt
+        dz = None
+        if not head:
+            dz = torch.empty(Pn, 256, device=dev)
+            ops.linear_dgrad(dz8, Wt, 32, 256, dz, mask_src=acts[7], mask_bits=bits[7], rows_dev=rd)
         dCAT = dE = None
         tmp_b = {}
         if fold is not None:
@@ -640,6 +652,11 @@
                     ops.linear_wgrad(dz, E, gW, tmp_b[0], 256, CNL_LDE, rows_dev=rd)
                     dE = torch.empty(Pn, CNL_LDE, device=dev)
                     ops.linear_dgrad(dz, Wt, 256, CNL_LDE, dE, rows_dev=rd)
+                elif i == 7 and head:
+                    inp = acts[6]
+                    ops.linear_wgrad_head(dz8, Wh, bits[7], inp, gW, gb, rows_dev=rd)
+                    dz = torch.empty(Pn, 256, device=dev)
+                    ops.linear_dgrad_head(dz8, Wh, bits[7], Wt, dz, mask_bits=bits[6], rows_dev=rd)
                 else:
                     inp = acts[i - 1]
                     ops.linear_wgrad(dz, inp, gW, gb, 256, 256, rows_dev=rd)
diff --git a/hosnerf_amd/ops.py b/hosnerf_amd/ops.py
--- a/hosnerf_amd/ops.py
+++ b/hosnerf_amd/ops.py
@@ -260,6 +260,37 @@
     _timed(f"gemm_wgrad[M={N},N={K},K={M}]", 2.0 * M * N * K, lambda: call(
         "hos_linear_wgrad", ptr(dY), dY.stride(0), ptr(X), X.stride(0), ptr(dW) + 4 * w_col0, dW.stride(0),
         ptr(db), M, N, K, splits, ptr(rows_dev, torch.int32)))
+
+
+def cnl_head_rows(M: int) -> bool:
+    return thin_dgrad_rows(M) and M % 32 == 0
+
+
+def linear_fwd_head(X: torch.Tensor, W: torch.Tensor, bias: torch.Tensor, out: torch.Tensor, Wh: torch.Tensor, bh: torch.Tensor,
+                    raw: torch.Tensor, relu_bits: Optional[torch.Tensor] = None, rows_dev: Optional[torch.Tensor] = None):
+    M = X.shape[0]
+    _timed(f"thin_fwd_head[M={M},N=256,K=256]", 2.0 * M * 256 * 260, lambda: call(
+        "hos_thin_linear_fwd_head", ptr(X), X.stride(0), ptr(W), W.stride(0), ptr(bias), ptr(out), out.stride(0),
+        ptr(Wh), Wh.stride(0), ptr(bh), ptr(raw), M, ptr(relu_bits, torch.int16), ptr(rows_dev, torch.int32)))
+    return raw
+
+
+def linear_dgrad_head(dZh: torch.Tensor, Wh: torch.Tensor, head_bits: torch.Tensor, W: torch.Tensor, out: torch.Tensor,
+                      mask_bits: Optional[torch.Tensor] = None, rows_dev: Optional[torch.Tensor] = None):
+    M = dZh.shape[0]
+    _timed(f"thin_dgrad_head[M={M},N=256,K=256]", 2.0 * M * 256 * 260, lambda: call(
+        "hos_thin_linear_dgrad_head", ptr(dZh), dZh.stride(0), ptr(Wh), Wh.stride(0), ptr(head_bits, torch.int16), ptr(W), W.stride(0),
+        ptr(mask_bits, torch.int16), ptr(out), out.stride(0), M, ptr(rows_dev, torch.int32)))
+    return out
+
+
+def linear_wgrad_head(dZh: torch.Tensor, Wh: torch.Tensor, head_bits: torch.Tensor, X: torch.Tensor, dW: torch.Tensor,
+                      db: Optional[torch.Tensor], rows_dev: Optional[torch.Tensor] = None):
+    M = dZh.shape[0]
+    ws = _bwd_workspace(dZh.device, M, 256, 256, False)
+    _timed(f"wgrad_tr_head[M=256,N=256,K={M}]", 2.0 * M * 256 * 260, lambda: call(
+        "hos_linear_wgrad_tr_head", ptr(dZh), dZh.stride(0), ptr(Wh), Wh.stride(0), ptr(head_bits, torch.int16), ptr(X), X.stride(0),
+        ptr(dW), dW.stride(0), ptr(db), M, ptr(ws), ws.numel(), ptr(rows_dev, torch.int32)))
 
 
 def linear_bwd_fused(dY: torch.Tensor, X: torch.Tensor, W: torch.Tensor, dW: torch.Tensor, db: Optional[torch.Tensor], N: int,
diff --git a/include/hosrender.h b/include/hosrender.h
--- a/include/hosrender.h
+++ b/include/hosrender.h
@@ -72,6 +72,16 @@
                         int M, int N, int K, int epilogue, void* relu_bits, const int32_t* rows_dev, hos_stream_t stream);
 int hos_thin_linear_dgrad(const float* dY, int lddy, const float* W, int ldw, int Npad, const float* mask, int ldmask,
                           const void* mask_bits, float* dX, int lddx, int M, int K, const int32_t* rows_dev, hos_stream_t stream);
+
+int hos_thin_linear_fwd_head(const float* X, int ldx, const float* W, int ldw, const float* bias, float* Y, int ldy,
+                             const float* Wh, int ldwh, const float* bh, float* raw, int M, void* relu_bits,
+                             const int32_t* rows_dev, hos_stream_t stream);
+int hos_thin_linear_dgrad_head(const float* dZh, int lddzh, const float* Wh, int ldwh, const void* head_bits,
+                               const float* W, int ldw, const void* mask_bits, float* dX, int lddx, int M,
+                               const int32_t* rows_dev, hos_stream_t stream);
+int hos_linear_wgrad_tr_head(const float* dZh, int lddzh, const float* Wh, int ldwh, const void* head_bits,
+                             const float* X, int ldx, float* dW, int lddw, float* db, int M, float* ws, int64_t ws_floats,
+                             const int32_t* rows_dev, hos_stream_t stream);
 
 int hos_canonical_fold_pack(const float* W0, int ld0, const float* b0, const float* W5, int ld5, const float* b5,
                             const float* embed, int n_out, int nf, int ne, int nh,
```

Measured after the change: 141,900, median of 6. About the same (+0.5%).
